# moxime/joint-vae

Hardware: AMD Instinct MI355X
Metric: training_images_per_sec (higher is better)
Workload: dtype f32

## Files before the change

include/jvae_hip.h:

```cpp
#ifndef JVAE_HIP_H
#define JVAE_HIP_H

#include <stddef.h>

#ifdef __cplusplus
extern "C" {
#endif

const char* jvae_version(void);

int jvae_gemm_f32(int M, int N, int K, int batch,
                  const float* A, long sAm, long sAk, long sAb,
                  const float* B, long sBk, long sBn, long sBb,
                  float* C, long sCm, long sCn, long sCb,
                  const float* bias, int bias_mode, int flags, int splitk, void* stream);

int jvae_splitk_fold_f32(const float* part, const float* bias, float* y, int S, long MN, int N, int relu, int accumulate,
                         void* stream);

size_t jvae_conv2d_workspace_bytes(int N, int Cin, int H, int W, int Cout, int KH, int KW, int S, int P, int OP,
                                   int transposed);
int jvae_conv2d_set_split_bf16(int mode);
int jvae_conv2d_set_split_shape16(int on);
int jvae_conv2d_out_shape(int H, int W, int KH, int KW, int S, int P, int OP, int transposed, int* OH, int* OW);
int jvae_conv2d_route(int dir, int layout, int bias, int stats, int y_f32, int aff_kind,
                      int N, int Cin, int H, int W, int Cout, int KH, int KW, int S, int P, int OP, int transposed,
                      int* kernel, int* swap, size_t* ws_bytes, int* splits, int* aff_ok);
const char* jvae_conv2d_kernel_name(int kernel);
int jvae_conv2d_fwd_f32(const float* x, const float* w, const float* bias, float* y,
                        int N, int Cin, int H, int W, int Cout, int KH, int KW, int S, int P, int OP, int transposed,
                        void* ws, size_t ws_bytes, void* stream);
int jvae_conv2d_stats_splits(int N, int Cin, int H, int W, int Cout, int KH, int KW, int S, int P, int OP, int transposed);
int jvae_conv2d_fwd_stats_f32(const float* x, const float* w, const float* bias, float* y, float* stats, int* nsplit,
                              int N, int Cin, int H, int W, int Cout, int KH, int KW, int S, int P, int OP, int transposed,
                              void* ws, size_t ws_bytes, void* stream);
int jvae_conv2d_dgrad_f32(const float* dy, const float* w, float* dx,
                          int N, int Cin, int H, int W, int Cout, int KH, int KW, int S, int P, int OP, int transposed,
                          void* ws, size_t ws_bytes, void* stream);
int jvae_conv2d_wgrad_f32(const float* x, const float* dy, float* dw, float* dbias, int accumulate,
                          int N, int Cin, int H, int W, int Cout, int KH, int KW, int S, int P, int OP, int transposed,
                          void* ws, size_t ws_bytes, void* stream);

int jvae_pack_cache_configure(void* buf, size_t bytes);
int jvae_pack_cache_begin(void* stream, long long owner, const void* const* weights, int n);
int jvae_pack_cache_end(void);
int jvae_pack_cache_pin(void);
int jvae_pack_cache_reset(void);
int jvae_pack_cache_stats(int* entries, long long* hits, long long* misses, long long* refreshes);

size_t jvae_channel_sum_workspace_bytes(int C);
int jvae_channel_sum_f32(const float* t, float* out, int N, int C, int P, int accumulate, void* ws, size_t ws_bytes,
                         void* stream);

size_t jvae_bn_workspace_bytes(int C);
int jvae_bn_plan(int N, int C, int P, int* nsplit, int* nchunk);
int jvae_image_range(int N, int parts, int j, int* nb, int* ne);
int jvae_bn_fwd_f32(const float* x, const float* gamma, const float* beta,
                    float* running_mean, float* running_var, long long* num_batches_tracked,
                    float* y, float* save_mean, float* save_invstd,
                    int N, int C, int P, float momentum, float eps, int training, int relu,
                    void* ws, size_t ws_bytes, void* stream);
int jvae_bn_fwd_ext_f32(const float* x, const float* gamma, const float* beta,
                        float* running_mean, float* running_var, long long* num_batches_tracked,
                        float* y, float* save_mean, float* save_invstd,
                        int N, int C, int P, float momentum, float eps, int training, int relu,
                        const float* ext_stats, int ext_nsplit, const float* ext_pivot,
                        void* ws, size_t ws_bytes, void* stream);
int jvae_bn_bwd_f32(const float* dy, const float* x, const float* gamma, const float* beta,
                    const float* save_mean, const float* save_invstd,
                    float* dx, float* dgamma, float* dbeta, int accumulate,
                    int N, int C, int P, int relu, void* ws, size_t ws_bytes, void* stream);
int jvae_bn_eval_bwd_f32(const float* dy, const float* x, const float* gamma, const float* beta,
                         const float* running_mean, const float* running_var, float* dx,
                         int N, int C, int P, float eps, int relu, void* stream);

int jvae_bn_finalize_f32(const float* x, const float* gamma, const float* beta,
                         float* running_mean, float* running_var, long long* num_batches_tracked,
                         float* save_mean, float* save_invstd, float* scale, float* shift,
                         int N, int C, int P, float momentum, float eps, int training,
                         const float* ext_stats, int ext_nsplit, const float* ext_pivot,
                         void* ws, size_t ws_bytes, void* stream);
int jvae_conv2d_affine_ok(int N, int Cin, int H, int W, int Cout, int KH, int KW, int S, int P, int OP, int transposed);
int jvae_conv2d_fwd_aff_f32(const float* x, const float* w, const float* bias, float* y, float* stats, int* nsplit,
                            const float* in_scale, const float* in_shift, int in_relu,
                            int N, int Cin, int H, int W, int Cout, int KH, int KW, int S, int P, int OP, int transposed,
                            void* ws, size_t ws_bytes, void* stream);
int jvae_conv2d_wgrad_aff_f32(const float* x, const float* dy, float* dw, float* dbias, int accumulate,
                              const float* in_scale, const float* in_shift, int in_relu,
                              int N, int Cin, int H, int W, int Cout, int KH, int KW, int S, int P, int OP, int transposed,
                              void* ws, size_t ws_bytes, void* stream);

int jvae_bn_sums_f32(const float* x, const float* pivot, float* sums, int N, int C, int P,
                     void* ws, size_t ws_bytes, void* stream);
int jvae_bn_fwd_sync_f32(const float* x, const float* gamma, const float* beta,
                         float* running_mean, float* running_var, long long* num_batches_tracked,
                         float* y, float* save_mean, float* save_invstd,
                         int N, int C, int P, float momentum, float eps, int relu,
                         const float* global_sums, const float* pivot, int world,
                         void* ws, size_t ws_bytes, void* stream);
int jvae_bn_bwd_sums_f32(const float* dy, const float* x, const float* gamma, const float* beta,
                         const float* save_mean, const float* save_invstd, float* local_sums,
                         int N, int C, int P, int relu, void* ws, size_t ws_bytes, void* stream);
int jvae_bn_bwd_sync_f32(const float* dy, const float* x, const float* gamma, const float* beta,
                         const float* save_mean, const float* save_invstd,
                         const float* local_sums, const float* global_sums, int world,
                         float* dx, float* dgamma, float* dbeta, int accumulate,
                         int N, int C, int P, int relu, void* stream);

int jvae_b8_pack_f32(const float* x, void* y, int N, int C, long HW, void* stream);
int jvae_b8_unpack_f32(const void* y, float* x, int N, int C, long HW, int accumulate, void* stream);
int jvae_conv2d_native_b8(int N, int Cin, int H, int W, int Cout, int KH, int KW, int S, int P, int OP, int transposed);
size_t jvae_conv2d_workspace_bytes_b8(int N, int Cin, int H, int W, int Cout, int KH, int KW, int S, int P, int OP,
                                      int transposed);
int jvae_conv2d_stats_splits_b8(int N, int Cin, int H, int W, int Cout, int KH, int KW, int S, int P, int OP, int transposed);
int jvae_conv2d_fwd_b8(const void* x, const float* w, const float* bias, void* y, int y_f32, float* stats, int* nsplit,
                       int N, int Cin, int H, int W, int Cout, int KH, int KW, int S, int P, int OP, int transposed,
                       void* ws, size_t ws_bytes, void* stream);
int jvae_conv2d_dgrad_b8(const void* dy, const float* w, void* dx,
                         int N, int Cin, int H, int W, int Cout, int KH, int KW, int S, int P, int OP, int transposed,
                         void* ws, size_t ws_bytes, void* stream);
int jvae_conv2d_wgrad_b8(const void* x, const void* dy, float* dw, float* dbias, int accumulate,
                         int N, int Cin, int H, int W, int Cout, int KH, int KW, int S, int P, int OP, int transposed,
                         void* ws, size_t ws_bytes, void* stream);
size_t jvae_bn_workspace_bytes_b8(int C);
int jvae_bn_plan_b8(int N, int C, long HW, int* nsplit, int* nchunk);
int jvae_bn_fwd_b8(const void* x, const float* gamma, const float* beta,
                   float* running_mean, float* running_var, long long* num_batches_tracked,
                   void* y, float* save_mean, float* save_invstd,
                   int N, int C, long HW, float momentum, float eps, int training, int relu,
                   const float* ext_stats, int ext_nsplit, const float* ext_pivot,
                   void* ws, size_t ws_bytes, void* stream);
int jvae_bn_bwd_b8(const void* dy, const void* x, const float* gamma, const float* beta,
                   const float* save_mean, const float* save_invstd,
                   void* dx, float* dgamma, float* dbeta, int accumulate,
                   int N, int C, long HW, int relu, void* ws, size_t ws_bytes, void* stream);
int jvae_bn_finalize_b8(const void* x, const float* gamma, const float* beta,
                        float* running_mean, float* running_var, long long* num_batches_tracked,
                        float* save_mean, float* save_invstd, float* coef,
                        int N, int C, long HW, float momentum, float eps, int training,
                        const float* ext_stats, int ext_nsplit, const float* ext_pivot,
                        void* ws, size_t ws_bytes, void* stream);
int jvae_bn_sums_b8(const void* x, const float* pivot, float* sums, int N, int C, long HW,
                    void* ws, size_t ws_bytes, void* stream);
int jvae_bn_fwd_sync_b8(const void* x, const float* gamma, const float* beta,
                        float* running_mean, float* running_var, long long* num_batches_tracked,
                        void* y, float* save_mean, float* save_invstd,
                        int N, int C, long HW, float momentum, float eps, int relu,
                        const float* global_sums, const float* pivot, int world,
                        void* ws, size_t ws_bytes, void* stream);
int jvae_bn_bwd_sums_b8(const void* dy, const void* x, const float* gamma, const float* beta,
                        const float* save_mean, const float* save_invstd, float* local_sums,
                        int N, int C, long HW, int relu, void* ws, size_t ws_bytes, void* stream);
int jvae_bn_bwd_sync_b8(const void* dy, const void* x, const float* gamma, const float* beta,
                        const float* save_mean, const float* save_invstd,
                        const float* local_sums, const float* global_sums, int world,
                        void* dx, float* dgamma, float* dbeta, int accumulate,
                        int N, int C, long HW, int relu, void* ws, size_t ws_bytes, void* stream);
int jvae_conv2d_affine_ok_b8(int N, int Cin, int H, int W, int Cout, int KH, int KW, int S, int P, int OP, int transposed);
int jvae_conv2d_fwd_aff_b8(const void* x, const float* w, const float* bias, void* y, int y_f32, float* stats, int* nsplit,
                           const float* in_scale, const float* in_shift, int in_relu,
                           int N, int Cin, int H, int W, int Cout, int KH, int KW, int S, int P, int OP, int transposed,
                           void* ws, size_t ws_bytes, void* stream);
int jvae_conv2d_wgrad_aff_b8(const void* x, const void* dy, float* dw, float* dbias, int accumulate,
                             const float* in_scale, const float* in_shift, int in_relu,
                             int N, int Cin, int H, int W, int Cout, int KH, int KW, int S, int P, int OP, int transposed,
                             void* ws, size_t ws_bytes, void* stream);
int jvae_relu_fwd_b8(const void* x, void* y, long units, void* stream);
int jvae_relu_bwd_b8(const void* dy, const void* y, void* dx, long units, void* stream);

int jvae_act_fwd_f32(const float* x, float* y, long n, int kind, void* stream);
int jvae_act_bwd_f32(const float* dy, const float* y, float* dx, long n, int kind, void* stream);

int jvae_dict_stats_f32(const float* means, float* dict, int C, int K, void* stream);
int jvae_latent_fwd_f32(const float* mu, const float* lv_raw, const float* eps, const long long* y,
                        const float* means, const float* T, const float* dict,
                        float* lv, float* z, float* kl, float* zdist, float* var_kl, float* dzdist,
                        int N, int K, int L, int C, int prior, int var_dim, float tau, float alpha, float w,
                        int sampled, int has_forced, float forced_lv, void* stream);
int jvae_latent_bwd_f32(const float* mu, const float* lv_raw, const float* lv, const float* eps, const long long* y,
                        const float* means, const float* T,
                        const float* gz, const float* g_kl, const float* g_zdist, const float* g_vkl,
                        const float* gmu_direct, const float* glv_direct,
                        float* gmu, float* glv_raw, float* gmeans, float* gT,
                        int N, int K, int L, int C, int prior, int var_dim, float tau, float alpha, float w,
                        int sampled, int has_forced, void* ws, size_t ws_bytes, void* stream);
int jvae_latent_fwd_wdev_f32(const float* mu, const float* lv_raw, const float* eps, const long long* y,
                             const float* means, const float* T, const float* dict,
                             float* lv, float* z, float* kl, float* zdist, float* var_kl, float* dzdist,
                             int N, int K, int L, int C, int prior, int var_dim, float tau, float alpha, float w,
                             int sampled, int has_forced, float forced_lv, const float* w_dev, void* stream);
int jvae_latent_bwd_wdev_f32(const float* mu, const float* lv_raw, const float* lv, const float* eps, const long long* y,
                             const float* means, const float* T,
                             const float* gz, const float* g_kl, const float* g_zdist, const float* g_vkl,
                             const float* gmu_direct, const float* glv_direct,
                             float* gmu, float* glv_raw, float* gmeans, float* gT,
                             int N, int K, int L, int C, int prior, int var_dim, float tau, float alpha, float w,
                             int sampled, int has_forced, const float* w_dev, void* ws, size_t ws_bytes, void* stream);
int jvae_latent_mixed_fwd_f32(const float* mu, const float* lv_raw, const float* eps, const long long* y,
                              const float* means_a, const float* T_a, const float* dict, const float* means_b, const float* T_b,
                              float* lv, float* z, float* kl, float* zdist, float* var_kl, float* dzdist,
                              int N, int K, int L, int split,
                              int C_a, int prior_a, int var_dim_a, float tau_a, float alpha_a,
                              int C_b, int prior_b, int var_dim_b, float tau_b, float alpha_b,
                              float w, int sampled, int has_forced, float forced_lv, void* stream);
int jvae_latent_mixed_bwd_f32(const float* mu, const float* lv_raw, const float* lv, const float* eps, const long long* y,
                              const float* means_a, const float* T_a, const float* means_b, const float* T_b,
                              const float* gz, const float* g_kl, const float* g_zdist, const float* g_vkl,
                              const float* gmu_direct, const float* glv_direct,
                              float* gmu, float* glv_raw, float* gmeans, float* gT,
                              int N, int K, int L, int split,
                              int C_a, int prior_a, int var_dim_a, float tau_a, float alpha_a,
                              int C_b, int prior_b, int var_dim_b, float tau_b, float alpha_b,
                              float w, int sampled, int has_forced, void* ws, size_t ws_bytes, void* stream);

int jvae_recon_fwd_f32(const float* x_reco, const float* x, const float* sigma, int sigma_is_log,
                       float* wmse, int L, int N, int D, void* stream);
int jvae_recon_bwd_f32(const float* x_reco, const float* x, const float* sigma, int sigma_is_log, const float* sigma_fwd,
                       const float* g_wmse, const float* wmse, float* g_x_reco, float* gsigma, int accumulate_sigma,
                       int L, int N, int D, void* ws, size_t ws_bytes, void* stream);

int jvae_mse_rows_fwd_f32(const float* rows, const float* x, float* wmse, int L, int N, int D, void* stream);
int jvae_mse_rows_bwd_f32(const float* rows, const float* x, const float* g_wmse, float* g_rows, int L, int N, int D, void* stream);

int jvae_elbo_fwd_f32(const float* wmse_s, const float* kl, const float* ce, const float* sigma, int sigma_is_log,
                      float* wmse, float* cross_x, float* total, float* mse, int L, int N, int D, float beta, float cw,
                      void* stream);
int jvae_elbo_bwd_f32(const float* g_wmse, const float* g_cx, const float* g_tot, const float* sigma, int sigma_is_log,
                      float* g_wmse_s, float* g_kl, float* g_ce, float* gsigma, int accumulate_sigma,
                      int L, int N, int D, float beta, float cw, void* ws, size_t ws_bytes, void* stream);
int jvae_elbo_fwd_wdev_f32(const float* wmse_s, const float* kl, const float* ce, const float* sigma, int sigma_is_log,
                           float* wmse, float* cross_x, float* total, float* mse, int L, int N, int D, float beta, float cw,
                           const float* cw_dev, void* stream);
int jvae_elbo_bwd_wdev_f32(const float* g_wmse, const float* g_cx, const float* g_tot, const float* sigma, int sigma_is_log,
                           float* g_wmse_s, float* g_kl, float* g_ce, float* gsigma, int accumulate_sigma,
                           int L, int N, int D, float beta, float cw, const float* cw_dev, void* ws, size_t ws_bytes,
                           void* stream);

int jvae_dropout_f32(const float* x, float* y, long n, float p, long seed, void* stream);
int jvae_dropout_dev_f32(const float* x, float* y, long n, float p, const long long* seed_dev, long salt, void* stream);

int jvae_iws_f32(const float* wmse_s, const float* eps, const float* log_var, const float* log_pz, const float* sigma,
                 int sigma_is_log, int L, int N, int K, int C, int D, float* rows, float* iws, void* stream);

int jvae_measures_f32(const float* sumsq_x, long nx, const float* wmse, const float* zdist, const float* var_kl, int N, int Nz,
                      const float* sigma, int sigma_is_log, const float* means, int C, int K, const int* flag,
                      const float* prev, int batch, float* out, void* stream);
int jvae_measures_dev_f32(const float* sumsq_x, long nx, const float* wmse, const float* zdist, const float* var_kl, int N, int Nz,
                          const float* sigma, int sigma_is_log, const float* means, int C, int K, const int* flag,
                          float* run, int* counter, void* stream);

int jvae_loss_sums_f32(const float* const* rows, const long* lens, int nrows, float* acc, void* stream);

int jvae_xent_fwd_f32(const float* logits, const long long* y, float* ce, int R, int N, int C, void* stream);
int jvae_xent_bwd_f32(const float* logits, const long long* y, const float* g_ce, float* g_logits, int R, int N, int C,
                      void* stream);

size_t jvae_sqnorm_workspace_bytes(void);
int jvae_sqnorm_accum_f32(const float* g, long n, float* acc, int reset, void* ws, size_t ws_bytes, void* stream);
int jvae_clip_scale_f32(float* g, long n, const float* sqnorm, float max_norm, void* stream);
int jvae_adam_step_f32(float* p, const float* g, float* m, float* v, long n,
                       float lr, float beta1, float beta2, float eps, float weight_decay, long step,
                       float max_norm, const float* sqnorm, int* nonfinite_flag, void* stream);
int jvae_adam_step_dev_f32(float* p, const float* g, float* m, float* v, long n, float* hyper, int advance,
                           float eps, float weight_decay, float max_norm, const float* sqnorm, int* nonfinite_flag,
                           void* stream);

int jvae_sgd_step_f32(float* p, const float* g, float* buf, long n, float lr, float momentum, int nesterov,
                      float weight_decay, int first_step, float max_norm, const float* sqnorm, int* nonfinite_flag,
                      void* stream);

int jvae_pool2d_out_shape(int H, int W, int K, int S, int P, int* OH, int* OW);
int jvae_pool2d_fwd_f32(const float* x, float* y, int* idx, long planes, int H, int W, int K, int S, int P, int mode,
                        void* stream);
int jvae_pool2d_bwd_f32(const float* dy, const int* idx, float* dx, long planes, int H, int W, int K, int S, int P,
                        int mode, void* stream);
int jvae_upsample_nearest_fwd_f32(const float* x, float* y, long planes, int H, int W, int scale, void* stream);
int jvae_upsample_nearest_bwd_f32(const float* dy, float* dx, long planes, int H, int W, int scale, void* stream);
int jvae_pool2d_fwd_b8(const void* x, void* y, int* idx, long blocks, int H, int W, int K, int S, int P, int mode, void* stream);
int jvae_pool2d_bwd_b8(const void* dy, const int* idx, void* dx, long blocks, int H, int W, int K, int S, int P, int mode,
                       void* stream);
int jvae_upsample_nearest_fwd_b8(const void* x, void* y, long blocks, int H, int W, int scale, void* stream);
int jvae_upsample_nearest_bwd_b8(const void* dy, void* dx, long blocks, int H, int W, int scale, void* stream);

int jvae_augment_u8_f32(const unsigned char* in, const unsigned char* flip, const int* dy, const int* dx,
                        float* out, int N, int C, int H, int W, int pad, int nhwc, void* stream);

int jvae_imageset_desc_words(void);
int jvae_imageset_batch_u8_f32(const unsigned char* data, const long long* idx, const long long* targets, const long long* lut,
                               const int* desc, const int* coef_h, const int* bounds_h, const int* coef_v, const int* bounds_v,
                               const unsigned char* flip, const int* dy, const int* dx, float* x, long long* y, long n, int N,
                               void* stream);

int jvae_imageset_mix_leaf_bytes(void);
int jvae_imageset_mixed_u8_f32(const void* leaves_host, const void* leaves_dev, int n_leaves, const int* leaf,
                               const long long* index, const long long* tag, const long long* pos, const float* u, int u_dims,
                               float* x, long long* tagout, long long* y, int N, int vec, void* stream);

size_t jvae_roc_workspace_bytes(int M, long n_in, long n_out);
int jvae_roc_curve_f32(const float* ins, const float* outs, const double* kept_tpr, const int* two_sided,
                       double* auc, double* kept_fpr, double* kept_tpr_out, double* thr_low, double* thr_up, int* status,
                       int M, long n_in, long n_out, int K, void* ws, size_t ws_bytes, void* stream);

int jvae_scod_scores_f32(const float* const* r_src, const float* const* r_aux, const float* const* g_src,
                         const float* const* g_alt, const int* kinds, const float* weights, const long long* y_est,
                         float* out, long out_stride, int M, int C, long N, int* status, void* stream);
size_t jvae_scod_workspace_bytes(int M, long n);
int jvae_scod_curve_f32(const float* scores, const long long* y_true, const long long* y_est, float* curves, double* figures,
                        int* status, int M, long n, long n_in, void* ws, size_t ws_bytes, void* stream);

int jvae_misclass_scores_f32(const float* src, const int* kinds, const float* temps, const int* rows, float* out,
                             int R, int C, long N, long out_stride, void* stream);
size_t jvae_misclass_split_workspace_bytes(long N);
int jvae_misclass_split_f32(const float* scores, const unsigned char* mask, float* out, int* n_correct, int M, long N,
                            void* ws, size_t ws_bytes, void* stream);
int jvae_misclass_confusion_f32(const float* scores, const unsigned char* mask, const double* thr, int* tp, int* fp,
                                int M, long N, int K, void* stream);

int jvae_odin_head_f32(const float* logits, const float* temps, float* scores, float* dlogits,
                       int F, int L, int N, int C, long stride_f, long stride_l, void* stream);
int jvae_odin_perturb_f32(float* acc, const float* g, const float* x, const float* eps, float* out, long numel, int E,
                          void* stream);
// ... 37 lines not shown
```

joint-vae_amd/csrc/gemm.hip:

```cpp
#include <stdlib.h>
#include "common.h"
#include "conv_x3.h"
#include "jvae_internal.h"
#include "conv_dispatch.h"

namespace {

constexpr int BK = 32;
constexpr int KQ = BK / 4;

struct GemmP {
    const float* A; long sAm, sAk, sAb;
    const float* B; long sBk, sBn, sBb;
    float* C; long sCm, sCn, sCb;
    const float* bias;
    int bias_mode;
    int bias_div;
    int M, N, K;
    int splitk;
    int kchunk;
    int flags;
    long sCsplit;
    int vecA, vecB;
    int xcd;
};

template <bool VEC>
__device__ __forceinline__ f32x4 load4(const float* p, long stride, int i0, int lim, bool row_ok) {
    f32x4 v = {0.f, 0.f, 0.f, 0.f};
    if (!row_ok) return v;
    if (VEC) {
        if (i0 + 3 < lim) return *reinterpret_cast<const f32x4*>(p);
    }
#pragma unroll
    for (int j = 0; j < 4; ++j)
        if (i0 + j < lim) v[j] = p[j * stride];
    return v;
}

template <int BM, int BN, bool AK, bool BNC>
__global__ __launch_bounds__(256) void gemm_kernel(GemmP p) {
    constexpr int LDA = BM + 4, LDB = BN + 4;
    constexpr int WM = BM / 2, WN = BN / 2;
    constexpr int TM = WM / 32, TN = WN / 32;
    constexpr int GA = BM * BK / 4 / 256;
    constexpr int GB = BN * BK / 4 / 256;
    __shared__ float As[BK * LDA];
    __shared__ float Bs[BK * LDB];

    const int tid = threadIdx.x, lane = tid & 63, wave = tid >> 6;
    const int wm0 = (wave >> 1) * WM, wn0 = (wave & 1) * WN;
    const int m0 = blockIdx.y * BM, n0 = blockIdx.x * BN;
    const int batch = blockIdx.z / p.splitk, split = blockIdx.z % p.splitk;
    const int kbeg = split * p.kchunk;
    const int kend = min(p.K, kbeg + p.kchunk);
    const float* A = p.A + (long)batch * p.sAb;
    const float* B = p.B + (long)batch * p.sBb;
    float* C = p.C + (long)batch * p.sCb + ((p.flags & 8) ? (long)split * p.sCsplit : 0L);

    f32x16 acc[TM][TN];
#pragma unroll
    for (int i = 0; i < TM; ++i)
#pragma unroll
        for (int j = 0; j < TN; ++j)
#pragma unroll
            for (int r = 0; r < 16; ++r) acc[i][j][r] = 0.f;

    f32x4 ra[GA], rb[GB];

    auto gload = [&](int k0) {
#pragma unroll
        for (int g = 0; g < GA; ++g) {
            if (AK) {
                const int kq = tid % KQ, row = tid / KQ + g * (256 / KQ);
                const int m = m0 + row, k = k0 + kq * 4;
                const float* src = A + (long)m * p.sAm + (long)k * p.sAk;
                ra[g] = p.vecA ? load4<true>(src, p.sAk, k, kend, m < p.M) : load4<false>(src, p.sAk, k, kend, m < p.M);
            } else {
                constexpr int GPR = BM / 4;
                const int mq = tid % GPR, kr = tid / GPR + g * (256 / GPR);
                const int m = m0 + mq * 4, k = k0 + kr;
                const float* src = A + (long)m * p.sAm + (long)k * p.sAk;
                ra[g] = p.vecA ? load4<true>(src, p.sAm, m, p.M, k < kend) : load4<false>(src, p.sAm, m, p.M, k < kend);
            }
        }
#pragma unroll
        for (int g = 0; g < GB; ++g) {
            if (BNC) {
                constexpr int GPR = BN / 4;
                const int nq = tid % GPR, kr = tid / GPR + g * (256 / GPR);
                const int n = n0 + nq * 4, k = k0 + kr;
                const float* src = B + (long)k * p.sBk + (long)n * p.sBn;
                rb[g] = p.vecB ? load4<true>(src, p.sBn, n, p.N, k < kend) : load4<false>(src, p.sBn, n, p.N, k < kend);
            } else {
                const int kq = tid % KQ, col = tid / KQ + g * (256 / KQ);
                const int n = n0 + col, k = k0 + kq * 4;
                const float* src = B + (long)k * p.sBk + (long)n * p.sBn;
                rb[g] = p.vecB ? load4<true>(src, p.sBk, k, kend, n < p.N) : load4<false>(src, p.sBk, k, kend, n < p.N);
            }
        }
    };
    auto lstore = [&]() {
#pragma unroll
        for (int g = 0; g < GA; ++g) {
            if (AK) {
                const int kq = tid % KQ, row = tid / KQ + g * (256 / KQ);
#pragma unroll
                for (int j = 0; j < 4; ++j) As[(kq * 4 + j) * LDA + row] = ra[g][j];
            } else {
                constexpr int GPR = BM / 4;
                const int mq = tid % GPR, kr = tid / GPR + g * (256 / GPR);
                *reinterpret_cast<f32x4*>(&As[kr * LDA + mq * 4]) = ra[g];
            }
        }
#pragma unroll
        for (int g = 0; g < GB; ++g) {
            if (BNC) {
                constexpr int GPR = BN / 4;
                const int nq = tid % GPR, kr = tid / GPR + g * (256 / GPR);
                *reinterpret_cast<f32x4*>(&Bs[kr * LDB + nq * 4]) = rb[g];
            } else {
                const int kq = tid % KQ, col = tid / KQ + g * (256 / KQ);
#pragma unroll
                for (int j = 0; j < 4; ++j) Bs[(kq * 4 + j) * LDB + col] = rb[g][j];
            }
        }
    };

    const int half = lane >> 5, l31 = lane & 31;
    if (kbeg < kend) gload(kbeg);
    for (int k0 = kbeg; k0 < kend; k0 += BK) {
        __syncthreads();
        lstore();
        __syncthreads();
        if (k0 + BK < kend) gload(k0 + BK);
#pragma unroll
        for (int kk = 0; kk < BK / 2; ++kk) {
            float a[TM], b[TN];
#pragma unroll
            for (int i = 0; i < TM; ++i) a[i] = As[(2 * kk + half) * LDA + wm0 + i * 32 + l31];
#pragma unroll
            for (int j = 0; j < TN; ++j) b[j] = Bs[(2 * kk + half) * LDB + wn0 + j * 32 + l31];
#pragma unroll
            for (int i = 0; i < TM; ++i)
#pragma unroll
                for (int j = 0; j < TN; ++j)
                    acc[i][j] = __builtin_amdgcn_mfma_f32_32x32x2f32(a[i], b[j], acc[i][j], 0, 0, 0);
        }
    }

    const bool lead = (split == 0) && !(p.flags & 8);
#pragma unroll
    for (int i = 0; i < TM; ++i)
#pragma unroll
        for (int j = 0; j < TN; ++j) {
            const int n = n0 + wn0 + j * 32 + l31;
            if (n >= p.N) continue;
            float bn = (p.bias_mode == 1 && lead) ? p.bias[n / p.bias_div] : 0.f;
#pragma unroll
            for (int r = 0; r < 16; ++r) {
                const int m = m0 + wm0 + i * 32 + (r & 3) + 8 * (r >> 2) + 4 * half;
                if (m >= p.M) continue;
                float v = acc[i][j][r] + bn;
                if (p.bias_mode == 2 && lead) v += p.bias[m];
                float* dst = C + (long)m * p.sCm + (long)n * p.sCn;
                if (p.flags & 8) {
                    *dst = v;
                } else if (p.flags & 4) {
                    atomicAdd(dst, v);
                } else {
                    if (p.flags & 1) v += *dst;
                    if (p.flags & 2) v = fmaxf(v, 0.f);
                    *dst = v;
                }
            }
        }
}

template <int BM, int BN>
int launch_tile(const GemmP& p, int batch, hipStream_t st) {
    dim3 grid(cdiv(p.N, BN), cdiv(p.M, BM), batch * p.splitk), block(256);
    const bool ak = (p.sAk == 1), bnc = (p.sBn == 1);
    if (ak && bnc)       hipLaunchKernelGGL((gemm_kernel<BM, BN, true, true>), grid, block, 0, st, p);
    else if (ak && !bnc) hipLaunchKernelGGL((gemm_kernel<BM, BN, true, false>), grid, block, 0, st, p);
    else if (!ak && bnc) hipLaunchKernelGGL((gemm_kernel<BM, BN, false, true>), grid, block, 0, st, p);
    else                 hipLaunchKernelGGL((gemm_kernel<BM, BN, false, false>), grid, block, 0, st, p);
    JVAE_LAUNCH_CHECK();
    return 0;
}

inline bool aligned16(const void* p) { return (reinterpret_cast<uintptr_t>(p) & 15) == 0; }

typedef __bf16 gx_bf16x8 __attribute__((ext_vector_type(8)));
typedef __bf16 gx_bf16x4 __attribute__((ext_vector_type(4)));
typedef unsigned int gx_u32x2 __attribute__((ext_vector_type(2)));
typedef unsigned int gx_u32x4 __attribute__((ext_vector_type(4)));
typedef __attribute__((address_space(3))) gx_bf16x4 gx_lds_bf16x4;
constexpr int BKX = 32;

__device__ __forceinline__ void gx_split4(const f32x4& v, gx_u32x2 (&out)[3]) {
#pragma unroll
    for (int j = 0; j < 2; ++j) {
        unsigned h, m, l;
        x3_split2(x3_f32x2{v[2 * j], v[2 * j + 1]}, h, m, l);
        out[0][j] = h; out[1][j] = m; out[2][j] = l;
    }
}

template <bool KC>
struct GxImg {
    static constexpr int PITCH = KC ? (BKX * 2 + 16) : (64 * 2 + 64);
    static constexpr int ROWS = KC ? 64 : BKX;
    static constexpr int BYTES = PITCH * ROWS;
};

template <bool AK, bool BNC, int DEPTH = 1>
__global__ __launch_bounds__(256, 4) void gemm_x3_kernel(GemmP p) {
    using IA = GxImg<AK>;
    using IB = GxImg<!BNC>;
    constexpr int BM = 64, BN = 64, G4 = BM * BKX / 4 / 256;
    constexpr int KQX = BKX / 4;
    extern __shared__ __attribute__((aligned(16))) unsigned char gx_lds[];
    unsigned char* As = gx_lds;
    unsigned char* Bs = gx_lds + 3 * IA::BYTES;

    const int tid = threadIdx.x, lane = tid & 63, wave = tid >> 6;
    const int half = lane >> 5, l31 = lane & 31;
    const int cg = (lane >> 4) & 1, q4 = (lane & 15) >> 2, pp = lane & 3;
    const int wm0 = (wave >> 1) * 32, wn0 = (wave & 1) * 32;
    unsigned bx = blockIdx.x, by = blockIdx.y, bz = blockIdx.z;
    if (p.xcd) {
        const unsigned lin = (unsigned)xcd_tile(bx + gridDim.x * (by + gridDim.y * bz), gridDim.x * gridDim.y * gridDim.z);
        bx = lin % gridDim.x; by = (lin / gridDim.x) % gridDim.y; bz = lin / (gridDim.x * gridDim.y);
    }
    const int m0 = by * BM, n0 = bx * BN;
    const int batch = bz / p.splitk, split = bz % p.splitk;
    const int kbeg = split * p.kchunk;
    const int kend = min(p.K, kbeg + p.kchunk);
    const float* A = p.A + (long)batch * p.sAb;
    const float* B = p.B + (long)batch * p.sBb;
    float* C = p.C + (long)batch * p.sCb + ((p.flags & 8) ? (long)split * p.sCsplit : 0L);

    f32x16 acc;
#pragma unroll
    for (int r = 0; r < 16; ++r) acc[r] = 0.f;
    f32x4 ra[DEPTH][G4], rb[DEPTH][G4];

    auto coordA = [&](int g, int k0, int* fast, int* slow) {
        if (AK) { *fast = k0 + (tid % KQX) * 4; *slow = m0 + tid / KQX + g * (256 / KQX); }
        else    { *fast = m0 + (tid % 16) * 4;  *slow = k0 + tid / 16 + g * 16; }
    };
    auto coordB = [&](int g, int k0, int* fast, int* slow) {
        if (BNC) { *fast = n0 + (tid % 16) * 4;  *slow = k0 + tid / 16 + g * 16; }
        else     { *fast = k0 + (tid % KQX) * 4; *slow = n0 + tid / KQX + g * (256 / KQX); }
    };
    auto okA = [&](int fast, int slow) { return AK ? (fast < kend && slow < p.M) : (fast + 3 < p.M && slow < kend); };
    auto okB = [&](int fast, int slow) { return BNC ? (fast + 3 < p.N && slow < kend) : (fast < kend && slow < p.N); };

    auto gload = [&](int st, int k0) {
#pragma unroll
        for (int g = 0; g < G4; ++g) {
            if constexpr (DEPTH > 1) {
                int f, sl;
                coordA(g, k0, &f, &sl);
                const float* sa = AK ? A + (long)sl * p.sAm + f : A + (long)sl * p.sAk + f;
                ra[st][g] = *reinterpret_cast<const f32x4*>(okA(f, sl) ? sa : A);
                coordB(g, k0, &f, &sl);
                const float* sb = BNC ? B + (long)sl * p.sBk + f : B + (long)sl * p.sBn + f;
                rb[st][g] = *reinterpret_cast<const f32x4*>(okB(f, sl) ? sb : B);
                continue;
            }
            if (AK) {
                const int kq = tid % KQX, row = tid / KQX + g * (256 / KQX);
                const int m = m0 + row, k = k0 + kq * 4;
                const float* src = A + (long)m * p.sAm + (long)k * p.sAk;
                ra[st][g] = p.vecA ? load4<true>(src, p.sAk, k, kend, m < p.M) : load4<false>(src, p.sAk, k, kend, m < p.M);
            } else {
                const int mq = tid % 16, kr = tid / 16 + g * 16;
                const int m = m0 + mq * 4, k = k0 + kr;
                const float* src = A + (long)m * p.sAm + (long)k * p.sAk;
                ra[st][g] = p.vecA ? load4<true>(src, p.sAm, m, p.M, k < kend) : load4<false>(src, p.sAm, m, p.M, k < kend);
            }
            if (BNC) {
                const int nq = tid % 16, kr = tid / 16 + g * 16;
                const int n = n0 + nq * 4, k = k0 + kr;
                const float* src = B + (long)k * p.sBk + (long)n * p.sBn;
                rb[st][g] = p.vecB ? load4<true>(src, p.sBn, n, p.N, k < kend) : load4<false>(src, p.sBn, n, p.N, k < kend);
            } else {
                const int kq = tid % KQX, col = tid / KQX + g * (256 / KQX);
                const int n = n0 + col, k = k0 + kq * 4;
                const float* src = B + (long)k * p.sBk + (long)n * p.sBn;
                rb[st][g] = p.vecB ? load4<true>(src, p.sBk, k, kend, n < p.N) : load4<false>(src, p.sBk, k, kend, n < p.N);
            }
        }
    };
    auto lstore = [&](int st, int k0) {
#pragma unroll
        for (int g = 0; g < G4; ++g) {
            const int fa = AK ? tid % KQX : tid % 16, sa_ = AK ? tid / KQX + g * (256 / KQX) : tid / 16 + g * 16;
            const int fb = BNC ? tid % 16 : tid % KQX, sb_ = BNC ? tid / 16 + g * 16 : tid / KQX + g * (256 / KQX);
            f32x4 va = ra[st][g], vb = rb[st][g];
            if constexpr (DEPTH > 1) {
                int f, sl;
                coordA(g, k0, &f, &sl);
                if (!okA(f, sl)) va = f32x4{0.f, 0.f, 0.f, 0.f};
                coordB(g, k0, &f, &sl);
                if (!okB(f, sl)) vb = f32x4{0.f, 0.f, 0.f, 0.f};
            }
            gx_u32x2 sa[3], sb[3];
            gx_split4(va, sa);
            gx_split4(vb, sb);
#pragma unroll
            for (int pl = 0; pl < 3; ++pl) {
                *reinterpret_cast<gx_u32x2*>(As + pl * IA::BYTES + sa_ * IA::PITCH + fa * 8) = sa[pl];
                *reinterpret_cast<gx_u32x2*>(Bs + pl * IB::BYTES + sb_ * IB::PITCH + fb * 8) = sb[pl];
            }
        }
    };
    auto frag = [&](const unsigned char* img, bool kc, int pitch, int r0, int ks) -> gx_bf16x8 {
        if (kc)
            return __builtin_bit_cast(gx_bf16x8, *reinterpret_cast<const gx_u32x4*>(img + (r0 + l31) * pitch + (ks * 16 + half * 8) * 2));
        const unsigned char* q = img + (ks * 16 + half * 8 + q4) * pitch + (r0 + cg * 16 + pp * 4) * 2;
        const gx_bf16x4 lo = __builtin_amdgcn_ds_read_tr16_b64_v4bf16((gx_lds_bf16x4*)q);
        const gx_bf16x4 hi = __builtin_amdgcn_ds_read_tr16_b64_v4bf16((gx_lds_bf16x4*)(q + 4 * pitch));
        return __builtin_shufflevector(lo, hi, 0, 1, 2, 3, 4, 5, 6, 7);
    };

    auto multiply = [&]() {
#pragma unroll
        for (int ks = 0; ks < BKX / 16; ++ks) {
            gx_bf16x8 a[3], b[3];
#pragma unroll
            for (int pl = 0; pl < 3; ++pl) {
                a[pl] = frag(As + pl * IA::BYTES, AK, IA::PITCH, wm0, ks);
                b[pl] = frag(Bs + pl * IB::BYTES, !BNC, IB::PITCH, wn0, ks);
            }
            constexpr int APL[6] = {0, 2, 1, 0, 1, 0}, BPL[6] = {2, 0, 1, 1, 0, 0};
#pragma unroll
            for (int t = 0; t < 6; ++t) acc = __builtin_amdgcn_mfma_f32_32x32x16_bf16(a[APL[t]], b[BPL[t]], acc, 0, 0, 0);
        }
    };
    if constexpr (DEPTH > 1) {
#pragma unroll
        for (int d = 0; d < DEPTH; ++d) gload(d, kbeg + d * BKX);
        const int nst = (kend - kbeg + BKX - 1) / BKX;
        int k0 = kbeg;
        for (int it = 0; it < nst / DEPTH; ++it, k0 += DEPTH * BKX) {
#pragma unroll
            for (int d = 0; d < DEPTH; ++d) {
                const int kk = k0 + d * BKX;
                __syncthreads();
                lstore(d, kk);
                __syncthreads();
                gload(d, kk + DEPTH * BKX);
                multiply();
            }
        }
#pragma unroll
        for (int d = 0; d < DEPTH - 1; ++d) {
            const int kk = k0 + d * BKX;
            if (kk < kend) {
                __syncthreads();
                lstore(d, kk);
                __syncthreads();
                multiply();
            }
        }
    } else {
        if (kbeg < kend) gload(0, kbeg);
        for (int k0 = kbeg; k0 < kend; k0 += BKX) {
            __syncthreads();
            lstore(0, k0);
            __syncthreads();
            if (k0 + BKX < kend) gload(0, k0 + BKX);
            multiply();
        }
    }

    const bool lead = (split == 0) && !(p.flags & 8);
    const int n = n0 + wn0 + l31;
    if (n >= p.N) return;
    const float bn = (p.bias_mode == 1 && lead) ? p.bias[n / p.bias_div] : 0.f;
#pragma unroll
    for (int r = 0; r < 16; ++r) {
        const int m = m0 + wm0 + (r & 3) + 8 * (r >> 2) + 4 * half;
        if (m >= p.M) continue;
        float v = acc[r] + bn;
        if (p.bias_mode == 2 && lead) v += p.bias[m];
        float* dst = C + (long)m * p.sCm + (long)n * p.sCn;
        if (p.flags & 8) {
            *dst = v;
        } else if (p.flags & 4) {
            atomicAdd(dst, v);
        } else {
            if (p.flags & 1) v += *dst;
            if (p.flags & 2) v = fmaxf(v, 0.f);
            *dst = v;
        }
    }
}

template <bool AK, bool BNC, int DEPTH>
int launch_x3_variant(const GemmP& p, int batch, hipStream_t st) {
    constexpr int LDS = 3 * (GxImg<AK>::BYTES + GxImg<!BNC>::BYTES);
    static bool attr_set = false;
    if (!attr_set) {
        hipError_t e = hipFuncSetAttribute(reinterpret_cast<const void*>(&gemm_x3_kernel<AK, BNC, DEPTH>),
                                           hipFuncAttributeMaxDynamicSharedMemorySize, LDS);
        if (e != hipSuccess) return (int)e;
        attr_set = true;
    }
    dim3 grid(cdiv(p.N, 64), cdiv(p.M, 64), batch * p.splitk), block(256);
    hipLaunchKernelGGL((gemm_x3_kernel<AK, BNC, DEPTH>), grid, block, LDS, st, p);
    JVAE_LAUNCH_CHECK();
    return 0;
}

template <bool AK, bool BNC>
int launch_x3_ab(const GemmP& p, int batch, hipStream_t st) {
    const bool deep = p.vecA && p.vecB && p.K % 4 == 0
                      && (AK || p.M % 4 == 0) && (!BNC || p.N % 4 == 0);
    if (deep) return launch_x3_variant<AK, BNC, 3>(p, batch, st);
    return launch_x3_variant<AK, BNC, 1>(p, batch, st);
}

int launch_x3(const GemmP& p0, int batch, hipStream_t st) {
    GemmP p = p0;
    p.xcd = 1;
    const bool ak = (p.sAk == 1), bnc = (p.sBn == 1);
    if (ak && bnc) return launch_x3_ab<true, true>(p, batch, st);
    if (ak) return launch_x3_ab<true, false>(p, batch, st);
    if (bnc) return launch_x3_ab<false, true>(p, batch, st);
    return launch_x3_ab<false, false>(p, batch, st);
}

inline bool gemm_x3_on(int K) {
    return K >= 64 && jvae_conv5_x3_enabled();
}

}

int jvae_gemm_launch(int M, int N, int K, int batch,
                     const float* A, long sAm, long sAk, long sAb,
                     const float* B, long sBk, long sBn, long sBb,
                     float* C, long sCm, long sCn, long sCb,
                     const float* bias, int bias_mode, int flags, int splitk, hipStream_t st) {
    return jvae_gemm_launch_ex(M, N, K, batch, A, sAm, sAk, sAb, B, sBk, sBn, sBb, C, sCm, sCn, sCb, bias, bias_mode, 1,
                               flags, splitk, st);
}

int jvae_gemm_launch_ex(int M, int N, int K, int batch,
                        const float* A, long sAm, long sAk, long sAb,
                        const float* B, long sBk, long sBn, long sBb,
                        float* C, long sCm, long sCn, long sCb,
                        const float* bias, int bias_mode, int bias_div, int flags, int splitk, hipStream_t st) {
    if (M <= 0 || N <= 0 || batch <= 0) return 0;
    if (K < 0 || !A || !B || !C) return JVAE_EINVAL;
    if (bias_mode && !bias) return JVAE_EINVAL;
    GemmP p;
    p.A = A; p.sAm = sAm; p.sAk = sAk; p.sAb = sAb;
    p.B = B; p.sBk = sBk; p.sBn = sBn; p.sBb = sBb;
    p.C = C; p.sCm = sCm; p.sCn = sCn; p.sCb = sCb;
    p.bias = bias; p.bias_mode = bias_mode; p.bias_div = bias_div > 0 ? bias_div : 1;
    p.M = M; p.N = N; p.K = K;
    if (splitk < 1) splitk = 1;
    int ktiles = cdiv(K, BK);
    if (splitk > ktiles) splitk = ktiles > 0 ? ktiles : 1;
    p.kchunk = cdiv(ktiles, splitk) * BK;
    splitk = K > 0 ? cdiv(K, p.kchunk) : 1;
    p.splitk = splitk;
    p.flags = flags & ~8;
    p.sCsplit = 0;
    if (splitk > 1) {
        if (flags & 2) return JVAE_EINVAL;
        p.flags |= 4;
    }
    const bool ak = (sAk == 1), bnc = (sBn == 1);
    p.vecA = aligned16(A) && (sAb % 4 == 0) && (ak ? (sAm % 4 == 0) : (sAm == 1 && sAk % 4 == 0));
    p.vecB = aligned16(B) && (sBb % 4 == 0) && (bnc ? (sBk % 4 == 0) : (sBk == 1 && sBn % 4 == 0));
    if (gemm_x3_on(K)) return launch_x3(p, batch, st);
    const long tiles128 = (long)cdiv(M, 128) * cdiv(N, 128) * batch * splitk;
    if (M > 64 && N > 64 && tiles128 >= 512) return launch_tile<128, 128>(p, batch, st);
    return launch_tile<64, 64>(p, batch, st);
}

int jvae_gemm_launch_part(int M, int N, int K, int batch,
                          const float* A, long sAm, long sAk, long sAb,
                          const float* B, long sBk, long sBn, long sBb,
                          float* part, long sCm, long sCn, long sCb, long sCsplit, int want_splits, int* splits,
                          hipStream_t st) {
    if (splits) *splits = 0;
    if (M <= 0 || N <= 0 || batch <= 0) return 0;
    if (K <= 0 || !A || !B || !part || !splits) return JVAE_EINVAL;
    GemmP p;
    p.A = A; p.sAm = sAm; p.sAk = sAk; p.sAb = sAb;
    p.B = B; p.sBk = sBk; p.sBn = sBn; p.sBb = sBb;
    p.C = part; p.sCm = sCm; p.sCn = sCn; p.sCb = sCb;
    p.bias = nullptr; p.bias_mode = 0; p.bias_div = 1;
    p.M = M; p.N = N; p.K = K;
    int splitk = want_splits < 1 ? 1 : want_splits;
    const int ktiles = cdiv(K, BK);
    if (splitk > ktiles) splitk = ktiles;
    p.kchunk = cdiv(ktiles, splitk) * BK;
    splitk = cdiv(K, p.kchunk);
    p.splitk = splitk;
    p.flags = 8;
    p.sCsplit = sCsplit;
    const bool ak = (sAk == 1), bnc = (sBn == 1);
    p.vecA = aligned16(A) && (sAb % 4 == 0) && (ak ? (sAm % 4 == 0) : (sAm == 1 && sAk % 4 == 0));
    p.vecB = aligned16(B) && (sBb % 4 == 0) && (bnc ? (sBk % 4 == 0) : (sBk == 1 && sBn % 4 == 0));
    *splits = splitk;
    if (gemm_x3_on(K)) return launch_x3(p, batch, st);
    return launch_tile<64, 64>(p, batch, st);
}

__global__ __launch_bounds__(256) void splitk_fold_kernel(const float* __restrict__ part, const float* __restrict__ bias,
                                                          float* __restrict__ y, int S, long MN, int N, int relu,
                                                          int accumulate, int bias_div) {
    for (long i = (long)blockIdx.x * blockDim.x + threadIdx.x; i < MN; i += (long)gridDim.x * blockDim.x) {
        float v = bias ? bias[(i / bias_div) % N] : 0.f;
        for (int s = 0; s < S; ++s) v += part[(long)s * MN + i];
        if (accumulate) v += y[i];
        y[i] = relu ? fmaxf(v, 0.f) : v;
    }
}

__global__ __launch_bounds__(256) void splitk_fold_qn_kernel(const float* __restrict__ part, const float* __restrict__ bias,
                                                             float* __restrict__ y, int S, int N, int Cs, int Ps) {
    const long total = (long)Ps * N * Cs;
    for (long i = (long)blockIdx.x * blockDim.x + threadIdx.x; i < total; i += (long)gridDim.x * blockDim.x) {
        const int cs = (int)(i % Cs);
        const long r = i / Cs;
        const int n = (int)(r % N), q = (int)(r / N);
        float v = bias ? bias[cs] : 0.f;
        for (int s = 0; s < S; ++s) v += part[(long)s * total + i];
        y[((long)n * Cs + cs) * Ps + q] = v;
    }
}

int jvae_splitk_fold_qn(const float* part, const float* bias, float* y, int S, int N, int Cs, int Ps, hipStream_t st) {
    const long total = (long)Ps * N * Cs;
    if (total == 0) return 0;
    const int blocks = (int)((total + 255) / 256 > 4096 ? 4096 : (total + 255) / 256);
    hipLaunchKernelGGL(splitk_fold_qn_kernel, dim3(blocks), dim3(256), 0, st, part, bias, y, S, N, Cs, Ps);
    JVAE_LAUNCH_CHECK();
    return 0;
}

int jvae_splitk_fold(const float* part, const float* bias, float* y, int S, long MN, int N, int relu, int accumulate,
                     hipStream_t st, int bias_div) {
    if (MN == 0) return 0;
    const int blocks = (int)((MN + 255) / 256 > 4096 ? 4096 : (MN + 255) / 256);
    hipLaunchKernelGGL(splitk_fold_kernel, dim3(blocks), dim3(256), 0, st, part, bias, y, S, MN, N, relu, accumulate,
                       bias_div > 0 ? bias_div : 1);
    JVAE_LAUNCH_CHECK();
    return 0;
}

extern "C" int jvae_splitk_fold_f32(const float* part, const float* bias, float* y, int S, long MN, int N, int relu,
                                    int accumulate, void* stream) {
    if (!part || !y || S < 1 || MN < 0 || N < 1) return JVAE_EINVAL;
    return jvae_splitk_fold(part, bias, y, S, MN, N, relu, accumulate, (hipStream_t)stream);
}

extern "C" int jvae_gemm_f32(int M, int N, int K, int batch,
                             const float* A, long sAm, long sAk, long sAb,
                             const float* B, long sBk, long sBn, long sBb,
                             float* C, long sCm, long sCn, long sCb,
                             const float* bias, int bias_mode, int flags, int splitk, void* stream) {
    return jvae_gemm_launch(M, N, K, batch, A, sAm, sAk, sAb, B, sBk, sBn, sBb, C, sCm, sCn, sCb,
                            bias, bias_mode, flags, splitk, (hipStream_t)stream);
}
```

joint-vae_amd/jvae_hip/lib.py:

```python
import ctypes
import os
from ctypes import c_char_p, c_float, c_int, c_long, c_longlong, c_size_t, c_void_p, POINTER

import torch

_HERE = os.path.dirname(os.path.abspath(__file__))
LIB_PATH = os.environ.get('JVAE_HIP_LIB') or os.path.join(_HERE, 'libjvae_hip.so')

_lib = None

P = c_void_p
_SIGS = {
    'jvae_version': (c_char_p, []),
    'jvae_gemm_f32': (c_int, [c_int] * 4 + [P, c_long, c_long, c_long] * 3 + [P, c_int, c_int, c_int, P]),
    'jvae_splitk_fold_f32': (c_int, [P, P, P, c_int, c_long, c_int, c_int, c_int, P]),
    'jvae_conv2d_workspace_bytes': (c_size_t, [c_int] * 11),
    'jvae_conv2d_set_split_bf16': (c_int, [c_int]),
    'jvae_conv2d_set_split_shape16': (c_int, [c_int]),
    'jvae_conv2d_out_shape': (c_int, [c_int] * 8 + [POINTER(c_int), POINTER(c_int)]),
    'jvae_conv2d_route': (c_int, [c_int] * 17 + [POINTER(c_int), POINTER(c_int), POINTER(c_size_t), POINTER(c_int), POINTER(c_int)]),
    'jvae_conv2d_kernel_name': (c_char_p, [c_int]),
    'jvae_conv2d_fwd_f32': (c_int, [P, P, P, P] + [c_int] * 11 + [P, c_size_t, P]),
    'jvae_conv2d_stats_splits': (c_int, [c_int] * 11),
    'jvae_conv2d_fwd_stats_f32': (c_int, [P, P, P, P, P, POINTER(c_int)] + [c_int] * 11 + [P, c_size_t, P]),
    'jvae_conv2d_dgrad_f32': (c_int, [P, P, P] + [c_int] * 11 + [P, c_size_t, P]),
    'jvae_conv2d_wgrad_f32': (c_int, [P, P, P, P, c_int] + [c_int] * 11 + [P, c_size_t, P]),
    'jvae_b8_pack_f32': (c_int, [P, P, c_int, c_int, c_long, P]),
    'jvae_b8_unpack_f32': (c_int, [P, P, c_int, c_int, c_long, c_int, P]),
    'jvae_conv2d_native_b8': (c_int, [c_int] * 11),
    'jvae_conv2d_workspace_bytes_b8': (c_size_t, [c_int] * 11),
    'jvae_conv2d_stats_splits_b8': (c_int, [c_int] * 11),
    'jvae_conv2d_fwd_b8': (c_int, [P, P, P, P, c_int, P, POINTER(c_int)] + [c_int] * 11 + [P, c_size_t, P]),
    'jvae_conv2d_dgrad_b8': (c_int, [P, P, P] + [c_int] * 11 + [P, c_size_t, P]),
    'jvae_conv2d_wgrad_b8': (c_int, [P, P, P, P, c_int] + [c_int] * 11 + [P, c_size_t, P]),
    'jvae_bn_workspace_bytes_b8': (c_size_t, [c_int]),
    'jvae_bn_plan_b8': (c_int, [c_int, c_int, c_long, POINTER(c_int), POINTER(c_int)]),
    'jvae_bn_fwd_b8': (c_int, [P] * 9 + [c_int, c_int, c_long, c_float, c_float, c_int, c_int, P, c_int, P, P, c_size_t, P]),
    'jvae_bn_bwd_b8': (c_int, [P] * 9 + [c_int, c_int, c_int, c_long, c_int, P, c_size_t, P]),
    'jvae_bn_finalize_b8': (c_int, [P] * 9 + [c_int, c_int, c_long, c_float, c_float, c_int, P, c_int, P, P, c_size_t, P]),
    'jvae_bn_sums_b8': (c_int, [P, P, P, c_int, c_int, c_long, P, c_size_t, P]),
    'jvae_bn_fwd_sync_b8': (c_int, [P] * 9 + [c_int, c_int, c_long, c_float, c_float, c_int, P, P, c_int, P, c_size_t, P]),
    'jvae_bn_bwd_sums_b8': (c_int, [P] * 7 + [c_int, c_int, c_long, c_int, P, c_size_t, P]),
    'jvae_bn_bwd_sync_b8': (c_int, [P] * 8 + [c_int, P, P, P, c_int, c_int, c_int, c_long, c_int, P, c_size_t, P]),
    'jvae_conv2d_affine_ok_b8': (c_int, [c_int] * 11),
    'jvae_conv2d_fwd_aff_b8': (c_int, [P, P, P, P, c_int, P, POINTER(c_int), P, P, c_int] + [c_int] * 11 + [P, c_size_t, P]),
    'jvae_conv2d_wgrad_aff_b8': (c_int, [P, P, P, P, c_int, P, P, c_int] + [c_int] * 11 + [P, c_size_t, P]),
    'jvae_relu_fwd_b8': (c_int, [P, P, c_long, P]),
    'jvae_relu_bwd_b8': (c_int, [P, P, P, c_long, P]),
    'jvae_bn_finalize_f32': (c_int, [P] * 10 + [c_int, c_int, c_int, c_float, c_float, c_int, P, c_int, P, P, c_size_t, P]),
    'jvae_conv2d_affine_ok': (c_int, [c_int] * 11),
    'jvae_conv2d_fwd_aff_f32': (c_int, [P, P, P, P, P, POINTER(c_int), P, P, c_int] + [c_int] * 11 + [P, c_size_t, P]),
    'jvae_conv2d_wgrad_aff_f32': (c_int, [P, P, P, P, c_int, P, P, c_int] + [c_int] * 11 + [P, c_size_t, P]),
    'jvae_pack_cache_configure': (c_int, [P, c_size_t]),
    'jvae_pack_cache_begin': (c_int, [P, c_longlong, P, c_int]),
    'jvae_pack_cache_end': (c_int, []),
    'jvae_pack_cache_pin': (c_int, []),
    'jvae_pack_cache_reset': (c_int, []),
    'jvae_pack_cache_stats': (c_int, [POINTER(c_int), POINTER(c_longlong), POINTER(c_longlong), POINTER(c_longlong)]),
    'jvae_channel_sum_workspace_bytes': (c_size_t, [c_int]),
    'jvae_channel_sum_f32': (c_int, [P, P, c_int, c_int, c_int, c_int, P, c_size_t, P]),
    'jvae_bn_workspace_bytes': (c_size_t, [c_int]),
    'jvae_bn_plan': (c_int, [c_int, c_int, c_int, POINTER(c_int), POINTER(c_int)]),
    'jvae_image_range': (c_int, [c_int, c_int, c_int, POINTER(c_int), POINTER(c_int)]),
    'jvae_bn_fwd_f32': (c_int, [P] * 9 + [c_int, c_int, c_int, c_float, c_float, c_int, c_int, P, c_size_t, P]),
    'jvae_bn_fwd_ext_f32': (c_int, [P] * 9 + [c_int, c_int, c_int, c_float, c_float, c_int, c_int, P, c_int, P, P, c_size_t, P]),
    'jvae_bn_sums_f32': (c_int, [P, P, P, c_int, c_int, c_int, P, c_size_t, P]),
    'jvae_bn_fwd_sync_f32': (c_int, [P] * 9 + [c_int, c_int, c_int, c_float, c_float, c_int, P, P, c_int, P, c_size_t, P]),
    'jvae_bn_bwd_sums_f32': (c_int, [P] * 7 + [c_int, c_int, c_int, c_int, P, c_size_t, P]),
    'jvae_bn_bwd_sync_f32': (c_int, [P] * 8 + [c_int, P, P, P, c_int, c_int, c_int, c_int, c_int, P]),
    'jvae_bn_bwd_f32': (c_int, [P] * 9 + [c_int, c_int, c_int, c_int, c_int, P, c_size_t, P]),
    'jvae_bn_eval_bwd_f32': (c_int, [P] * 7 + [c_int, c_int, c_int, c_float, c_int, P]),
    'jvae_act_fwd_f32': (c_int, [P, P, c_long, c_int, P]),
    'jvae_act_bwd_f32': (c_int, [P, P, P, c_long, c_int, P]),
    'jvae_dict_stats_f32': (c_int, [P, P, c_int, c_int, P]),
    'jvae_latent_fwd_f32': (c_int, [P] * 13 + [c_int] * 6 + [c_float] * 3 + [c_int, c_int, c_float, P]),
    'jvae_latent_bwd_f32': (c_int, [P] * 17 + [c_int] * 6 + [c_float] * 3 + [c_int, c_int, P, c_size_t, P]),
    'jvae_latent_fwd_wdev_f32': (c_int, [P] * 13 + [c_int] * 6 + [c_float] * 3 + [c_int, c_int, c_float, P, P]),
    'jvae_latent_bwd_wdev_f32': (c_int, [P] * 17 + [c_int] * 6 + [c_float] * 3 + [c_int, c_int, P, P, c_size_t, P]),
    'jvae_latent_mixed_fwd_f32': (c_int, [P] * 15 + [c_int] * 4 + ([c_int] * 3 + [c_float] * 2) * 2
                                  + [c_float, c_int, c_int, c_float, P]),
    'jvae_latent_mixed_bwd_f32': (c_int, [P] * 19 + [c_int] * 4 + ([c_int] * 3 + [c_float] * 2) * 2
                                  + [c_float, c_int, c_int, P, c_size_t, P]),
    'jvae_recon_fwd_f32': (c_int, [P, P, P, c_int, P, c_int, c_int, c_int, P]),
    'jvae_recon_bwd_f32': (c_int, [P, P, P, c_int, P, P, P, P, P, c_int, c_int, c_int, c_int, P, c_size_t, P]),
    'jvae_mse_rows_fwd_f32': (c_int, [P, P, P, c_int, c_int, c_int, P]),
    'jvae_mse_rows_bwd_f32': (c_int, [P, P, P, P, c_int, c_int, c_int, P]),
    'jvae_elbo_fwd_f32': (c_int, [P, P, P, P, c_int, P, P, P, P, c_int, c_int, c_int, c_float, c_float, P]),
    'jvae_elbo_bwd_f32': (c_int, [P, P, P, P, c_int, P, P, P, P, c_int, c_int, c_int, c_int, c_float, c_float, P, c_size_t, P]),
    'jvae_elbo_fwd_wdev_f32': (c_int, [P, P, P, P, c_int, P, P, P, P, c_int, c_int, c_int, c_float, c_float, P, P]),
    'jvae_elbo_bwd_wdev_f32': (c_int, [P, P, P, P, c_int, P, P, P, P, c_int, c_int, c_int, c_int, c_float, c_float, P, P, c_size_t, P]),
    'jvae_measures_dev_f32': (c_int, [P, c_long, P, P, P, c_int, c_int, P, c_int, P, c_int, c_int, P, P, P, P]),
    'jvae_loss_sums_f32': (c_int, [P, P, c_int, P, P]),
    'jvae_measures_f32': (c_int, [P, c_long, P, P, P, c_int, c_int, P, c_int, P, c_int, c_int, P, P, c_int, P, P]),
    'jvae_dropout_f32': (c_int, [P, P, c_long, c_float, c_long, P]),
    'jvae_dropout_dev_f32': (c_int, [P, P, c_long, c_float, P, c_long, P]),
    'jvae_iws_f32': (c_int, [P, P, P, P, P, c_int, c_int, c_int, c_int, c_int, c_int, P, P, P]),
    'jvae_xent_fwd_f32': (c_int, [P, P, P, c_int, c_int, c_int, P]),
    'jvae_xent_bwd_f32': (c_int, [P, P, P, P, c_int, c_int, c_int, P]),
    'jvae_augment_u8_f32': (c_int, [P, P, P, P, P, c_int, c_int, c_int, c_int, c_int, c_int, P]),
    'jvae_imageset_desc_words': (c_int, []),
    'jvae_imageset_batch_u8_f32': (c_int, [P] * 4 + [POINTER(c_int)] + [P] * 9 + [c_long, c_int, P]),
    'jvae_imageset_mix_leaf_bytes': (c_int, []),
    'jvae_imageset_mixed_u8_f32': (c_int, [P, P, c_int] + [P] * 5 + [c_int] + [P] * 3 + [c_int, c_int, P]),
    'jvae_sqnorm_workspace_bytes': (c_size_t, []),
    'jvae_sqnorm_accum_f32': (c_int, [P, c_long, P, c_int, P, c_size_t, P]),
    'jvae_clip_scale_f32': (c_int, [P, c_long, P, c_float, P]),
    'jvae_adam_step_dev_f32': (c_int, [P, P, P, P, c_long, P, c_int, c_float, c_float, c_float, P, P, P]),
    'jvae_adam_step_f32': (c_int, [P, P, P, P, c_long] + [c_float] * 5 + [c_long, c_float, P, P, P]),
    'jvae_sgd_step_f32': (c_int, [P, P, P, c_long, c_float, c_float, c_int, c_float, c_int, c_float, P, P, P]),
    'jvae_pool2d_out_shape': (c_int, [c_int] * 5 + [POINTER(c_int), POINTER(c_int)]),
    'jvae_pool2d_fwd_f32': (c_int, [P, P, P, c_long] + [c_int] * 6 + [P]),
    'jvae_pool2d_bwd_f32': (c_int, [P, P, P, c_long] + [c_int] * 6 + [P]),
    'jvae_upsample_nearest_fwd_f32': (c_int, [P, P, c_long, c_int, c_int, c_int, P]),
    'jvae_upsample_nearest_bwd_f32': (c_int, [P, P, c_long, c_int, c_int, c_int, P]),
    'jvae_pool2d_fwd_b8': (c_int, [P, P, P, c_long] + [c_int] * 6 + [P]),
    'jvae_pool2d_bwd_b8': (c_int, [P, P, P, c_long] + [c_int] * 6 + [P]),
    'jvae_upsample_nearest_fwd_b8': (c_int, [P, P, c_long, c_int, c_int, c_int, P]),
    'jvae_upsample_nearest_bwd_b8': (c_int, [P, P, c_long, c_int, c_int, c_int, P]),
    'jvae_roc_workspace_bytes': (c_size_t, [c_int, c_long, c_long]),
    'jvae_roc_curve_f32': (c_int, [P] * 10 + [c_int, c_long, c_long, c_int, P, c_size_t, P]),
    'jvae_scod_scores_f32': (c_int, [P] * 8 + [c_long, c_int, c_int, c_long, P, P]),
    'jvae_scod_workspace_bytes': (c_size_t, [c_int, c_long]),
    'jvae_scod_curve_f32': (c_int, [P] * 6 + [c_int, c_long, c_long, P, c_size_t, P]),
    'jvae_misclass_scores_f32': (c_int, [P] * 5 + [c_int, c_int, c_long, c_long, P]),
    'jvae_misclass_split_workspace_bytes': (c_size_t, [c_long]),
    'jvae_misclass_split_f32': (c_int, [P, P, P, P, c_int, c_long, P, c_size_t, P]),
    'jvae_misclass_confusion_f32': (c_int, [P] * 5 + [c_int, c_long, c_int, P]),
    'jvae_odin_head_f32': (c_int, [P, P, P, P, c_int, c_int, c_int, c_int, c_long, c_long, P]),
    'jvae_odin_perturb_f32': (c_int, [P, P, P, P, P, c_long, c_int, P]),
    'jvae_wim_scores_f32': (c_int, [P, P, P, c_int, P, P, c_int, P, c_long, c_int, c_long, P, P]),
    'jvae_group_tally_f32': (c_int, [P, P, P, P, c_int, c_int, c_int, P]),
    'jvae_prior_sample_f32': (c_int, [P] * 6 + [c_long, c_int, c_int, c_float, c_int, P]),
    'jvae_image_grid_f32': (c_int, [P, P, P, P, c_int, P, P] + [c_int] * 5 + [P]),
    'jvae_class_posterior_f32': (c_int, [P] * 5 + [c_int, P, P, c_long, c_int, c_int, c_int, P]),
    'jvae_latent_mi_workspace_bytes': (c_size_t, [c_int, c_int, c_long]),
    'jvae_latent_mi_f32': (c_int, [P, P, P, c_int, c_int, c_int, c_int, c_long, P, c_size_t, P]),
    'jvae_aggregate_scores_f32': (c_int, [P, P, c_int, c_int, P, c_int, P, P, P, P, c_int, c_int, c_long, P, P]),
    'jvae_cascade_mse_workspace_bytes': (c_size_t, [c_int, c_long, c_long]),
    'jvae_cascade_mse_f32': (c_int, [P, P, c_int, P, c_int, c_long, c_long, P, c_size_t, P]),
    'jvae_iterate_prior_f32': (c_int, [P, P, c_int, c_int, c_long, P]),
    'jvae_latent_moments_workspace_bytes': (c_size_t, [c_int, c_int, c_int]),
    'jvae_latent_moments_f32': (c_int, [P, P, P, P, P, c_int, c_int, c_int, P, c_size_t, P]),
    'jvae_nearest_centroid_f32': (c_int, [P, P, P, P, c_long, c_int, c_int, P]),
    'jvae_histogram_f32': (c_int, [P, P, P, P, P, c_long, c_int, c_int, P]),
}


class JvaeHipError(RuntimeError):
    pass


def load():
    global _lib
    if _lib is not None:
        return _lib
    if not os.path.exists(LIB_PATH):
        raise JvaeHipError(f'{LIB_PATH} is missing: build it with `python -c "import __graft_entry__ as g; g.build()"` '
                           'or `make -C joint-vae_amd/csrc` (there is no CPU/PyTorch fallback)')
    lib = ctypes.CDLL(LIB_PATH)
    for name, (res, args) in _SIGS.items():
        fn = getattr(lib, name)
        fn.restype = res
        fn.argtypes = args
    _lib = lib
    return lib


def exported_symbols():
    return list(_SIGS)


_ERR = {-1: 'invalid argument', -2: 'unsupported configuration', -3: 'workspace too small'}


def check(rc, what):
    if rc != 0:
        msg = _ERR.get(rc, f'hipError_t {rc}')
        raise JvaeHipError(f'{what} failed: {msg}')


_raw_stream = getattr(torch._C, '_cuda_getCurrentRawStream', None)


def stream_ptr(device_index=None):
    if _raw_stream is not None:
        return _raw_stream(torch.cuda.current_device() if device_index is None else device_index)
    return torch.cuda.current_stream().cuda_stream


def ptr(t):
    if t is None:
        return None
    if not t.is_cuda:
        raise JvaeHipError('jvae_hip ops need tensors resident on the GPU (no CPU fallback); got device '
                           + str(t.device))
    if not t.is_contiguous():
        raise JvaeHipError('jvae_hip ops need contiguous tensors')
    return t.data_ptr()


_workspaces = {}
_side_streams = {}


def side_stream(device):
    idx = device.index if device.index is not None else torch.cuda.current_device()
    st = _side_streams.get(idx)
    if st is None:
        _side_streams[idx] = st = torch.cuda.Stream(device=idx)
    return st


def join_side_stream(device=None):
    for idx, st in _side_streams.items():
        if device is None or device.index in (None, idx):
            torch.cuda.current_stream(idx).wait_stream(st)


def workspace(nbytes, device):
    idx = device.index if device.index is not None else torch.cuda.current_device()
    key = (idx, stream_ptr(idx))
    ws = _workspaces.get(key)
    if ws is None or ws.numel() < nbytes:
        _workspaces[key] = ws = torch.empty(max(int(nbytes), 1 << 20), dtype=torch.uint8, device=device)
    return ws


PACK_CACHE_BYTES = int(os.environ.get('JVAE_PACK_CACHE_MB', '64')) << 20
_pack_cache = {}
span_depth = 0
span_hold = 0


def pack_cache_begin(weights, device):
    if not PACK_CACHE_BYTES:
        return
    lib = load()
    idx = device.index if device.index is not None else torch.cuda.current_device()
    if idx not in _pack_cache:
        if _pack_cache:
            check(lib.jvae_pack_cache_configure(None, 0), 'jvae_pack_cache_configure')
            _pack_cache[idx] = None
        else:
            buf = torch.empty(PACK_CACHE_BYTES + 256, dtype=torch.uint8, device=device)
            off = (-buf.data_ptr()) % 256
            _pack_cache[idx] = buf
            check(lib.jvae_pack_cache_configure(buf.data_ptr() + off, PACK_CACHE_BYTES), 'jvae_pack_cache_configure')
    if _pack_cache[idx] is None:
        return
    addrs = tuple(w.data_ptr() for w in weights)
    arr = (ctypes.c_void_p * max(len(addrs), 1))(*addrs)
    check(lib.jvae_pack_cache_begin(stream_ptr(idx), hash(addrs), arr, len(addrs)), 'jvae_pack_cache_begin')


def pack_cache_end():
    if _lib is not None and _pack_cache:
        _lib.jvae_pack_cache_end()


def pack_cache_pin():
    if _lib is not None and _pack_cache and PACK_CACHE_BYTES:
        _lib.jvae_pack_cache_pin()


def pack_cache_stats():
    lib = load()
    e, h, m, r = c_int(), c_longlong(), c_longlong(), c_longlong()
    lib.jvae_pack_cache_stats(ctypes.byref(e), ctypes.byref(h), ctypes.byref(m), ctypes.byref(r))
    return {'entries': e.value, 'hits': h.value, 'misses': m.value, 'refreshes': r.value}
```

joint-vae_amd/jvae_hip/ops.py:

```python
import collections
import contextlib
import ctypes
import math
from ctypes import byref, c_int, c_size_t

import numpy as np
import torch

from . import lib as L

RELU, SIGMOID, IDENT, LEAKY = 1, 2, 0, 3
BN_ACT = {IDENT: 0, RELU: 1, LEAKY: 2}
OVERLAP_WGRAD = True
ACT_KIND = {'relu': RELU, 'sigmoid': SIGMOID, 'linear': IDENT, 'leaky': LEAKY, None: IDENT}


def _c(t):
    return t if t.is_contiguous() else t.contiguous()


def _f32(t, what):
    if t.dtype != torch.float32:
        raise L.JvaeHipError(f'{what}: fp32 expected, got {t.dtype}')
    return t


def _grad_slot(param):
    if param is None or not isinstance(param, torch.nn.Parameter):
        return None
    g = param.grad
    if g is None or not g.is_contiguous() or g.dtype != torch.float32 or g.shape != param.shape or not g.is_cuda:
        return None
    return g


def _join_after_backward():
    torch.autograd.Variable._execution_engine.queue_callback(L.join_side_stream)


def _close_span_after_backward():
    if not L.span_hold:
        torch.autograd.Variable._execution_engine.queue_callback(L.pack_cache_end)


def gemm(M, N, K, A, sA, B, sB, C, sC, bias=None, bias_mode=0, flags=0, splitk=1, batch=1):
    lib = L.load()
    rc = lib.jvae_gemm_f32(M, N, K, batch, L.ptr(A), *sA, L.ptr(B), *sB, L.ptr(C), *sC,
                           L.ptr(bias), bias_mode, flags, splitk, L.stream_ptr())
    L.check(rc, 'jvae_gemm_f32')


def channel_sum(t, N, C, P, out=None, accumulate=False):
    lib = L.load()
    if out is None:
        out = torch.empty(C, device=t.device, dtype=torch.float32)
    ws = L.workspace(lib.jvae_channel_sum_workspace_bytes(C), t.device)
    L.check(lib.jvae_channel_sum_f32(L.ptr(t), L.ptr(out), N, C, P, int(accumulate), L.ptr(ws), ws.numel(), L.stream_ptr()),
            'channel_sum')
    return out


def _linear_split(R, O, I):
    tiles = ((R + 63) // 64) * ((O + 63) // 64)
    if tiles >= 128 or I < 512:
        return 1
    for S in (32, 16, 8, 4, 2):
        if tiles * S <= 1024 and I % S == 0 and I // S >= 128:
            return S
    return 1


class _Linear(torch.autograd.Function):

    @staticmethod
    def forward(ctx, x, w, b, act):
        x2 = _c(_f32(x, 'linear').reshape(-1, x.shape[-1]))
        w_in = w
        w = _c(w)
        R, I = x2.shape
        O = w.shape[0]
        y = torch.empty((R, O), device=x.device, dtype=torch.float32)
        S = _linear_split(R, O, I)
        if S > 1:
            part = torch.empty((S, R, O), device=x.device, dtype=torch.float32)
            Ks = I // S
            gemm(R, O, Ks, x2, (I, 1, Ks), w, (1, I, Ks), part, (O, 1, R * O), batch=S)
            L.check(L.load().jvae_splitk_fold_f32(L.ptr(part), L.ptr(b), L.ptr(y), S, R * O, O, int(act == RELU), 0,
                                                  L.stream_ptr()), 'jvae_splitk_fold_f32')
        else:
            gemm(R, O, I, x2, (I, 1, 0), w, (1, I, 0), y, (O, 1, 0), bias=b, bias_mode=1 if b is not None else 0,
                 flags=2 if act == RELU else 0)
        if act in (SIGMOID, LEAKY):
            L.check(L.load().jvae_act_fwd_f32(L.ptr(y), L.ptr(y), y.numel(), act, L.stream_ptr()), 'act_fwd')
        ctx.save_for_backward(x2, w, y if act != IDENT else None)
        ctx.act = act
        ctx.has_bias = b is not None
        ctx.xshape = x.shape
        ctx.w_ref, ctx.b_ref = w_in, b
        return y.reshape(*x.shape[:-1], O)

    @staticmethod
    def backward(ctx, gy):
        x2, w, y = ctx.saved_tensors
        lib = L.load()
        R, I = x2.shape
        O = w.shape[0]
        gy = _c(gy.reshape(R, O))
        if ctx.act != IDENT:
            g = torch.empty_like(gy)
            L.check(lib.jvae_act_bwd_f32(L.ptr(gy), L.ptr(y), L.ptr(g), gy.numel(), ctx.act, L.stream_ptr()), 'act_bwd')
            gy = g
        gx = gw = gb = None
        if ctx.needs_input_grad[0]:
            gx = torch.empty((R, I), device=gy.device, dtype=torch.float32)
            gemm(R, I, O, gy, (O, 1, 0), w, (I, 1, 0), gx, (I, 1, 0))
            gx = gx.reshape(ctx.xshape)
        if ctx.needs_input_grad[1]:
            slot = _grad_slot(ctx.w_ref)
            gw = slot if slot is not None else torch.zeros((O, I), device=gy.device, dtype=torch.float32)
            S = _linear_split(O, I, R)
            if S > 1:
                part = torch.empty((S, O, I), device=gy.device, dtype=torch.float32)
                Rs = R // S
                gemm(O, I, Rs, gy, (1, O, Rs * O), x2, (I, 1, Rs * I), part, (I, 1, O * I), batch=S)
                L.check(lib.jvae_splitk_fold_f32(L.ptr(part), None, L.ptr(gw), S, O * I, I, 0, 1, L.stream_ptr()),
                        'jvae_splitk_fold_f32')
            else:
                gemm(O, I, R, gy, (1, O, 0), x2, (I, 1, 0), gw, (I, 1, 0), flags=1)
            if slot is not None:
                gw = None
        if ctx.has_bias and ctx.needs_input_grad[2]:
            slot = _grad_slot(ctx.b_ref)
            if slot is not None:
                channel_sum(gy, R, O, 1, out=slot, accumulate=True)
            else:
                gb = channel_sum(gy, R, O, 1)
        return gx, gw, gb, None


def linear(x, w, b=None, act=IDENT):
    return _Linear.apply(x, w, b, act)


_GEOM_CACHE = {}


def _geom_query(name, geom):
    key = (name, geom)
    r = _GEOM_CACHE.get(key)
    if r is None:
        _GEOM_CACHE[key] = r = getattr(L.load(), name)(*geom)
    return r


class ConvSpec:
    __slots__ = ('cin', 'cout', 'k', 's', 'p', 'op', 'transposed')

    def __init__(self, cin, cout, k, s, p, op=0, transposed=False):
        self.cin, self.cout, self.k, self.s, self.p, self.op, self.transposed = cin, cout, k, s, p, op, bool(transposed)

    def out_hw(self, H, W):
        key = ('hw', self.k, self.s, self.p, self.op, self.transposed, H, W)
        r = _GEOM_CACHE.get(key)
        if r is None:
            oh, ow = c_int(), c_int()
            rc = L.load().jvae_conv2d_out_shape(H, W, self.k, self.k, self.s, self.p, self.op, int(self.transposed),
                                                byref(oh), byref(ow))
            L.check(rc, 'jvae_conv2d_out_shape')
            _GEOM_CACHE[key] = r = (oh.value, ow.value)
        return r

    def geom(self, N, H, W):
        return (N, self.cin, H, W, self.cout, self.k, self.k, self.s, self.p, self.op, int(self.transposed))


def _conv_ws(geom, device):
    nbytes = _geom_query('jvae_conv2d_workspace_bytes', geom)
    ws = L.workspace(nbytes, device)
    return ws, ws.numel()


def conv_fwd_raw(x, w, b, spec):
    N, _, H, W = x.shape
    oh, ow = spec.out_hw(H, W)
    y = torch.empty((N, spec.cout, oh, ow), device=x.device, dtype=torch.float32)
    geom = spec.geom(N, H, W)
    ws, nb = _conv_ws(geom, x.device)
    rc = L.load().jvae_conv2d_fwd_f32(L.ptr(x), L.ptr(w), L.ptr(b), L.ptr(y), *geom, L.ptr(ws), nb, L.stream_ptr())
    L.check(rc, 'jvae_conv2d_fwd_f32')
    return y


def conv_fwd_stats_raw(x, w, b, spec):
    lib = L.load()
    N, _, H, W = x.shape
    geom = spec.geom(N, H, W)
    cap = _geom_query('jvae_conv2d_stats_splits', geom)
    if cap <= 0:
        return conv_fwd_raw(x, w, b, spec), None, 0
    oh, ow = spec.out_hw(H, W)
    y = torch.empty((N, spec.cout, oh, ow), device=x.device, dtype=torch.float32)
    stats = torch.empty((spec.cout * cap * 2,), device=x.device, dtype=torch.float32)
    ws, nb = _conv_ws(geom, x.device)
    ns = c_int(0)
    rc = lib.jvae_conv2d_fwd_stats_f32(L.ptr(x), L.ptr(w), L.ptr(b), L.ptr(y), L.ptr(stats), byref(ns), *geom,
                                       L.ptr(ws), nb, L.stream_ptr())
    L.check(rc, 'jvae_conv2d_fwd_stats_f32')
    return y, (stats if ns.value > 0 else None), ns.value


def conv_affine_ok(spec, N, H, W):
    return bool(_geom_query('jvae_conv2d_affine_ok', spec.geom(N, H, W)))


ConvRoute = collections.namedtuple('ConvRoute', 'kernel swap ws splits aff_ok')
ROUTE_DIR = {'fwd': 1, 'dgrad': 2, 'wgrad': 4}
ROUTE_LAYOUT = {'f32': 0, 'b8': 1}


def conv_route(spec, N, H, W, direction, layout='f32', bias=False, stats=False, y_f32=False, aff=0):
    lib = L.load()
    k, sw, ns, ok, ws = c_int(), c_int(), c_int(), c_int(), c_size_t()
    rc = lib.jvae_conv2d_route(ROUTE_DIR[direction], ROUTE_LAYOUT[layout], int(bias), int(stats), int(y_f32), int(aff),
                               *spec.geom(N, H, W), byref(k), byref(sw), byref(ws), byref(ns), byref(ok))
    L.check(rc, 'jvae_conv2d_route')
    return ConvRoute(lib.jvae_conv2d_kernel_name(k.value).decode(), bool(sw.value), ws.value, ns.value, bool(ok.value))


class LaunchProbe:

    def __init__(self, match):
        self.match, self.events, self.armed = match, [], False

    def times_ms(self):
        return [a.elapsed_time(b) for a, b in self.events]


FWD_AFF_PROBE = None


def conv_fwd_aff_raw(x, w, b, spec, aff, want_stats):
    lib = L.load()
    N, _, H, W = x.shape
    geom = spec.geom(N, H, W)
    oh, ow = spec.out_hw(H, W)
    y = torch.empty((N, spec.cout, oh, ow), device=x.device, dtype=torch.float32)
    stats, ns = None, c_int(0)
    if want_stats:
        cap = _geom_query('jvae_conv2d_stats_splits', geom)
        if cap > 0:
            stats = torch.empty((spec.cout * cap * 2,), device=x.device, dtype=torch.float32)
    ws, nb = _conv_ws(geom, x.device)
    probe = FWD_AFF_PROBE
    timed = probe is not None and probe.armed and probe.match(spec, N, H)
    if timed:
        ev = (torch.cuda.Event(enable_timing=True), torch.cuda.Event(enable_timing=True))
        ev[0].record()
    rc = lib.jvae_conv2d_fwd_aff_f32(L.ptr(x), L.ptr(w), L.ptr(b), L.ptr(y), L.ptr(stats), byref(ns),
                                     L.ptr(aff[0]), L.ptr(aff[1]), int(aff[2]), *geom, L.ptr(ws), nb, L.stream_ptr())
    if timed:
        ev[1].record()
        probe.events.append(ev)
    L.check(rc, 'jvae_conv2d_fwd_aff_f32')
    return y, (stats if ns.value > 0 else None), ns.value


def conv_dgrad_raw(gy, w, spec, xshape):
    N, _, H, W = xshape
    gx = torch.empty(xshape, device=gy.device, dtype=torch.float32)
    geom = spec.geom(N, H, W)
    ws, nb = _conv_ws(geom, gy.device)
    rc = L.load().jvae_conv2d_dgrad_f32(L.ptr(gy), L.ptr(w), L.ptr(gx), *geom, L.ptr(ws), nb, L.stream_ptr())
    L.check(rc, 'jvae_conv2d_dgrad_f32')
    return gx


def conv_wgrad_raw(x, gy, spec, wshape, want_bias, w_slot=None, b_slot=None, aff=None):
    N, _, H, W = x.shape
    inplace = w_slot is not None and (b_slot is not None or not want_bias)
    gw = w_slot if inplace else torch.empty(wshape, device=x.device, dtype=torch.float32)
    gb = None
    if want_bias:
        gb = b_slot if inplace else torch.empty(spec.cout, device=x.device, dtype=torch.float32)
    geom = spec.geom(N, H, W)
    ws, nb = _conv_ws(geom, x.device)
    if aff is not None:
        rc = L.load().jvae_conv2d_wgrad_aff_f32(L.ptr(x), L.ptr(gy), L.ptr(gw), L.ptr(gb), int(inplace),
                                                L.ptr(aff[0]), L.ptr(aff[1]), int(aff[2]), *geom, L.ptr(ws), nb,
                                                L.stream_ptr())
    else:
        rc = L.load().jvae_conv2d_wgrad_f32(L.ptr(x), L.ptr(gy), L.ptr(gw), L.ptr(gb), int(inplace), *geom, L.ptr(ws), nb,
                                            L.stream_ptr())
    L.check(rc, 'jvae_conv2d_wgrad_f32')
    return (None, None) if inplace else (gw, gb)


FWD, DGRAD, WGRAD = 1, 2, 4


class Layout:
    sfx = '_f32'
    ws_sfx = ''
    acts = BN_ACT

    def dims(self, x, C):
        N, C = x.shape[0], x.shape[1]
        return N, C, x.numel() // max(N * C, 1)

    def coef_width(self, C):
        return C

    def prep(self, x, what):
        return _c(_f32(x, what))

    def to_f32(self, t, C):
        return t

    def from_f32(self, t):
        return t

    def native(self, spec, N, H, W):
        return FWD | DGRAD | WGRAD

    def affine_ok(self, spec, N, H, W):
        return conv_affine_ok(spec, N, H, W)

    def conv_fwd(self, x, w, b, spec, want_stats, aff, out_f32):
        if aff is not None:
            return conv_fwd_aff_raw(x, w, b, spec, aff, want_stats)
        if want_stats:
            return conv_fwd_stats_raw(x, w, b, spec)
        return conv_fwd_raw(x, w, b, spec), None, 0

    def conv_dgrad(self, gy, w, spec, N, H, W):
        return conv_dgrad_raw(gy, w, spec, (N, spec.cin, H, W))

    def conv_wgrad(self, *args):
        return conv_wgrad_raw(*args)

    def bn(self, name, *args, ws=None):
        name += self.sfx
        extra = () if ws is None else (L.ptr(ws), ws.numel())
        L.check(getattr(L.load(), name)(*args, *extra, L.stream_ptr()), name)

    def bn_workspace(self, C, device):
        return L.workspace(getattr(L.load(), 'jvae_bn_workspace_bytes' + self.ws_sfx)(C), device)

    def bn_fwd(self, *args, ext, ws):
        if ext[0] is None:
            self.bn('jvae_bn_fwd', *args, ws=ws)
        else:
            self.bn('jvae_bn_fwd_ext', *args, *ext, ws=ws)

    def coef_args(self, coef):
        return L.ptr(coef[0]), L.ptr(coef[1])

    def bn_bwd_sync(self, *args, ws):
        self.bn('jvae_bn_bwd_sync', *args)


F32 = Layout()


def layout_of(t):
    return _b8.B8 if _b8.is_b8(t) else F32


class _Conv(torch.autograd.Function):

    @staticmethod
    def forward(ctx, x, w, b, spec, dead_bias, stats_out, aff, out_f32):
        lay = layout_of(x)
        x = lay.prep(x, 'conv')
        if not L.span_depth:
            L.pack_cache_end()
        ctx.w_ref, ctx.b_ref = w, b
        w = _c(w)
        native = lay.native(spec, x.shape[0], x.shape[2], x.shape[3])
        if aff is not None and (native & (FWD | WGRAD)) != FWD | WGRAD:
            raise L.JvaeHipError('a deferred BatchNorm needs native forward and weight-gradient kernels (conv_affine_ok)')
        want_stats = stats_out is not None
        if native & FWD:
            y, st, ns = lay.conv_fwd(x, w, b, spec, want_stats, aff, out_f32)
        else:
            y, st, ns = F32.conv_fwd(lay.to_f32(x, spec.cin), w, b, spec, want_stats, None, False)
            y = y if out_f32 else lay.from_f32(y)
        if want_stats:
            stats_out['stats'], stats_out['nsplit'], stats_out['pivot'] = st, ns, b
        ctx.save_for_backward(x, w)
        ctx.lay, ctx.native, ctx.spec, ctx.out_f32, ctx.aff = lay, native, spec, out_f32, aff
        ctx.has_bias = b is not None
        ctx.dead_bias = dead_bias
        return y

    @staticmethod
    def backward(ctx, gy):
        x, w = ctx.saved_tensors
        lay, spec = ctx.lay, ctx.spec
        N, H, W = x.shape[0], x.shape[2], x.shape[3]
        gys = {F32 if ctx.out_f32 else lay: _c(gy)}

        def gy_in(want):
            if want not in gys:
                have, g = next(iter(gys.items()))
                gys[want] = want.from_f32(g) if have is F32 else have.to_f32(g, spec.cout)
            return gys[want]
        gx = gw = gb = None
        _close_span_after_backward()
        want_b = ctx.has_bias and ctx.needs_input_grad[2] and not ctx.dead_bias
        wgrad = ctx.needs_input_grad[1] or want_b
        on_side = False
        if wgrad:
            w_slot = _grad_slot(ctx.w_ref)
            b_slot = _grad_slot(ctx.b_ref) if want_b else None
            on_side = (OVERLAP_WGRAD and ctx.needs_input_grad[0] and w_slot is not None
                       and (b_slot is not None or not want_b))
        if ctx.needs_input_grad[0]:
            dl = lay if ctx.native & DGRAD else F32
            gyd = gy_in(dl)
        if on_side:
            side = L.side_stream(x.device)
            side.wait_stream(torch.cuda.current_stream(x.device))
        if ctx.needs_input_grad[0]:
            gx = dl.conv_dgrad(gyd, w, spec, N, H, W)
            gx = gx if dl is lay else lay.from_f32(gx)
        if wgrad:
            with torch.cuda.stream(side) if on_side else contextlib.nullcontext():
                wl = lay if ctx.native & WGRAD else F32
                xw = x if wl is lay else lay.to_f32(x, spec.cin)
                gw, gb = wl.conv_wgrad(xw, gy_in(wl), spec, w.shape, want_b, w_slot, b_slot, ctx.aff)
            if on_side:
                for t in (x, xw, *gys.values(), *(ctx.aff[:2] if ctx.aff is not None else ())):
                    t.record_stream(side)
                _join_after_backward()
        if ctx.dead_bias and ctx.has_bias and ctx.needs_input_grad[2] and _grad_slot(ctx.b_ref) is None:
            gb = torch.zeros_like(ctx.b_ref)
        return gx, gw, gb, None, None, None, None, None


def conv2d(x, w, b, spec, dead_bias=False, stats_out=None, aff=None, out_f32=False):
    return _Conv.apply(x, w, b, spec, dead_bias, stats_out, aff, out_f32)


def _ext_args(ext, training):
# ... 1624 lines not shown
```

joint-vae_amd/module/vae_layers/layers.py:

```python
import logging
import math

import numpy as np
import torch
from torch import nn
from torch.nn import Parameter

from jvae_hip import ops
from jvae_compat import texify_str
from module.priors import build_prior
from .misc import activation_layers, ACT_OF_MODULE


def _sigma_kind(is_rmse, coded, learned, decay):
    for kind, on in (('rmse', is_rmse), ('coded', coded), ('learned', learned), ('decayed', decay)):
        if on:
            return kind
    return 'fixed'


class Sigma(Parameter):

    @staticmethod
    def __new__(cls, value=None, sdim=1, input_dim=False, learned=False, is_rmse=False, is_log=False, **_):
        if value is None:
            assert is_rmse or input_dim, 'a Sigma needs a value unless it follows the rmse or is coded'
        stored_as_log = bool(is_log or learned or input_dim)
        if is_rmse or (input_dim and value is None):
            start = 0.
        else:
            start = float(value)
        shape = (sdim,) if isinstance(sdim, int) else tuple(sdim)
        with np.errstate(divide='ignore'):
            init = float(np.log(start)) if stored_as_log else start
        return super().__new__(cls, torch.full(shape, init), requires_grad=bool(learned or input_dim))

    def __init__(self, value=None, learned=False, is_rmse=False, sdim=1, input_dim=False, reach=1, decay=0,
                 max_step=None, sigma0=None, is_log=False):
        if learned:
            assert not is_rmse and not decay, 'a learned sigma neither follows the rmse nor decays'
        follows = bool(decay) or is_rmse
        public = dict(is_rmse=is_rmse,
                      sigma0=sigma0 if (sigma0 is not None or is_rmse) else value,
                      learned=learned,
                      input_dim=input_dim,
                      is_log=learned or is_log or input_dim,
                      decay=1 if is_rmse else decay,
                      reach=reach if follows else None,
                      max_step=max_step,
                      sdim=sdim)
        self._rmse = np.nan
        self.__dict__.update(public)
        self._output_dim = None
        if input_dim:
            self._output_dim = input_dim if sdim != 1 else (1,) * len(input_dim)

    def __deepcopy__(self, memo):
        twin = Sigma.__new__(Sigma, value=1.0, sdim=self.sdim, learned=self.requires_grad)
        twin.__dict__.update(self.__dict__)
        twin.data = self.data.clone()
        memo[id(self)] = twin
        return twin

    coded = property(lambda self: bool(self.input_dim))
    per_dim = property(lambda self: self.sdim != 1)
    output_dim = property(lambda self: self._output_dim)
    kind = property(lambda self: _sigma_kind(self.is_rmse, self.coded, self.learned, self.decay))

    @property
    def value(self):
        with torch.no_grad():
            squares = (2 * self.data).exp() if self.is_log else self.data * self.data
            return float(squares.mean().sqrt())

    def host_params(self, value):
        listed = {k: v for k, v in vars(self).items() if k[:1] != '_'}
        listed['value'] = value
        return listed

    @property
    def params(self):
        return self.host_params(self.value)

    def update(self, rmse=None, v=None):
        assert rmse is None or v is None
        if v is not None:
            extra = v.dim() - self.dim()
            assert extra >= 0
            self.data = v.mean(tuple(range(extra))) if extra else v
        elif rmse is not None:
            self._rmse = rmse
            if self.kind in ('rmse', 'decayed'):
                step = self.decay * (self.reach * rmse - self.data)
                if self.max_step:
                    step = torch.clamp(torch.as_tensor(step), -self.max_step, self.max_step)
                self.data += step

    def _describe(self):
        kind = self.kind
        if kind == 'rmse':
            return 'rmse' if self._rmse is np.nan else 'rmse ({:g})'.format(self._rmse)
        if kind == 'coded':
            return 'coded ' + ('mask' if self.per_dim else 'scalar')
        if kind == 'learned':
            return '{:g}->rmse[l] ({:g})'.format(self.sigma0, self.value)
        if kind == 'fixed':
            return '{:g}'.format(self.value if self.dim() and self.numel() > 1 else float(self.data))
        target = ('' if self.reach == 1 else '{:g}*'.format(self.reach)) + 'rmse'
        limit = '<{:g}'.format(self.max_step) if self.max_step else ''
        return '{:g}->{}[-{:g}*{}]'.format(self.sigma0, target, self.decay, limit)

    def __str__(self):
        return self._describe()

    def __format__(self, spec):
        tail = spec[-1:] if spec else ''
        if tail in ('f', 'g', 'e'):
            return format(self.value, spec)
        if tail == 'x':
            return texify_str(self._describe(), num=True)
        if tail == 'i':
            letter = {'rmse': 'e', 'learned': 'l', 'coded': 'C' if self.per_dim else 'c'}.get(self.kind)
            if letter:
                return letter
        return self._describe()

    def __repr__(self):
        if self.kind == 'rmse':
            return 'Sigma will be RMSE'
        text = super().__repr__()
        if self.decay:
            text = '{}, decaying to {}*mse with rate {})'.format(text[:-1], self.reach, self.decay)
        return text


def draw_epsilon(sampling_size, shape, device, distribution='gaussian'):
    size = (sampling_size + 1,) + tuple(shape)
    if distribution == 'gaussian':
        eps = torch.randn(size, device=device)
    else:
        eps = (torch.rand(size, device=device) - 0.5) * math.sqrt(12)
    eps[0] = 0
    return eps


class Sampling(nn.Module):

    def __init__(self, latent_dim, sampling_size=1, sampling=True, distribution='gaussian', **kwargs):
        assert distribution in ('gaussian', 'uniform'), '{} for sampling unknown'.format(distribution)
        super().__init__(**kwargs)
        self.distribution = distribution
        self.sampling_size = sampling_size
        self.is_sampled = sampling

    def forward(self, z_mean, z_log_var, epsilon=None):
        K = z_mean.shape[-1]
        if epsilon is None:
            epsilon = draw_epsilon(self.sampling_size, z_log_var.shape, z_mean.device, self.distribution)
        mu2 = z_mean.reshape(-1, K)
        n = mu2.shape[0]
        labels = torch.zeros(n, dtype=torch.int64, device=z_mean.device)
        means = torch.zeros((1, K), device=z_mean.device)
        T = torch.ones(1, device=z_mean.device)
        _, z, _, _, _, _ = ops.latent(mu2, z_log_var.reshape(-1, K), epsilon.reshape(epsilon.shape[0], n, K), labels,
                                      means, T, sampled=bool(self.is_sampled))
        return z.reshape(epsilon.shape), epsilon[1:]

    def __repr__(self):
        if not self.is_sampled:
            return 'Deactivated, returns mean'
        return 'Sampling({}, L={})'.format(self.distribution, self.sampling_size)


class HipLinear(nn.Linear):

    def forward(self, x, act=ops.IDENT):
        return ops.linear(x, self.weight, self.bias, act)


class DenseStack(nn.Sequential):

    def forward(self, x):
        mods = list(self)
        i = 0
        while i < len(mods):
            m = mods[i]
            nxt = mods[i + 1] if i + 1 < len(mods) else None
            if isinstance(m, HipLinear) and type(nxt) in ACT_OF_MODULE:
                x = m(x, ACT_OF_MODULE[type(nxt)])
                i += 2
            else:
                x = m(x)
                i += 1
        return x


class HipDropout(nn.Module):

    _STRIDE = 0x9E3779B97F4A7C15 & (2 ** 62 - 1)

    def __init__(self, p=0.5):
        super().__init__()
        if not 0. <= p < 1.:
            raise ValueError('dropout probability has to be in [0, 1), got {}'.format(p))
        self.p = float(p)
        self._seed = None

    def _next_seed(self, device):
        if self._seed is None or self._seed.device != device:
            first = int(torch.randint(0, 2 ** 61, (1,)))
            if torch.distributed.is_available() and torch.distributed.is_initialized():
                first += torch.distributed.get_rank() * 1_000_003
            self._seed = torch.tensor([first], dtype=torch.int64, device=device)
        now = self._seed.clone()
        self._seed += self._STRIDE % (2 ** 31)
        return now

    def forward(self, x):
        if not self.training or self.p == 0.:
            if not x.is_cuda:
                raise ops.L.JvaeHipError('jvae_hip ops need tensors resident on the GPU (no CPU fallback)')
            return x
        return ops.dropout(x, self.p, self._next_seed(x.device))

    def extra_repr(self):
        return f'p={self.p}'


class Encoder(nn.Module):

    def __init__(self, input_shape, num_labels, representation='rgb', y_is_coded=False, latent_dim=32,
                 intermediate_dims=[64], name='encoder', dropout=False, activation='relu', sampling_size=10,
                 sampling=True, sigma_output_dim=0, forced_variance=False, prior={}, **kwargs):
        super().__init__(**kwargs)
        self.name = name
        self.y_is_coded = y_is_coded
        self.input_shape = input_shape
        self.num_labels = num_labels
        self.forced_variance = forced_variance
        self._sampling_size = sampling_size
        width = int(np.prod(input_shape)) + num_labels * bool(y_is_coded)
        trunk = []
        for d in intermediate_dims:
            trunk += [HipLinear(width, d), activation_layers[activation]()]
            if dropout:
                trunk.append(HipDropout(p=dropout))
            width = d
        self.dense_projs = DenseStack(*trunk)
        self.dense_mean = HipLinear(width, latent_dim)
        self.dense_log_var = HipLinear(width, latent_dim)
        self.sigma_output_dim = sigma_output_dim
        if sigma_output_dim:
            self.sigma = HipLinear(width, int(np.prod(sigma_output_dim)))

        noise = 'uniform' if prior.get('distribution', 'gaussian') == 'uniform' else 'gaussian'
        self.sampling = Sampling(latent_dim, sampling_size, sampling, distribution=noise)
        prior['dim'] = latent_dim
        self.prior = build_prior(**prior)
        logging.debug('Built %s', self.prior)
        self.mixed_prior = None

    @property
    def sampling_size(self):
        return self._sampling_size

    @sampling_size.setter
    def sampling_size(self, v):
        self._sampling_size = v
        self.sampling.sampling_size = v

    def capacity(self):
        m = self.prior.mean
        C = self.num_labels
        d2 = torch.cdist(m, m).pow(2)
        return math.log(C) - torch.exp(-d2 / 4).sum(0).log().sum() / C

    def dict_min_distance(self):
        m = self.prior.mean
        C = self.num_labels
        guard = 2 * m.norm(dim=1).max() * torch.eye(C, device=m.device)
        return (torch.cdist(m, m) + guard).min()

    def heads(self, x, y=None):
        u = x if y is None else torch.cat((x, y), dim=-1)
        u = self.dense_projs(u)
        return u, self.dense_mean(u), (None if self.forced_variance else self.dense_log_var(u))

    def encode(self, x, y_onehot, labels, kl_var_weighting=1., epsilon=None):
        u, mu, lv_raw = self.heads(x, y_onehot)
        K = mu.shape[-1]
        batch = mu.shape[:-1]
        mu2 = mu.reshape(-1, K)
        n = mu2.shape[0]
        pr = self.prior
        if epsilon is None:
            epsilon = draw_epsilon(self._sampling_size, mu.shape, mu.device, self.sampling.distribution)
        lab, means, T = pr._kernel_operands(labels if pr.conditional else None, n, mu.device)
        forced = math.log(self.forced_variance) if self.forced_variance else None
        raw2 = mu2 if lv_raw is None else lv_raw.reshape(-1, K)
        if self.mixed_prior is None:
            lv, z, kl, dist, vkl, dzd = ops.latent(mu2, raw2, epsilon.reshape(epsilon.shape[0], n, K), lab, means, T,
                                                   prior=pr.distribution, var_dim=pr.var_dim, tau=pr._tau,
                                                   alpha=pr._alpha_k, w=kl_var_weighting,
                                                   sampled=bool(self.sampling.is_sampled), forced_lv=forced)
        else:
            other, split = self.mixed_prior
            if not pr.conditional:
                raise NotImplementedError('a mixed prior needs the class-conditional prior in place')
            _, means_b, T_b = other._kernel_operands(labels if other.conditional else None, n, mu.device)
            describe = ops.latent_prior
            lv, z, kl, dist, vkl, dzd = ops.latent_mixed(
                mu2, raw2, epsilon.reshape(epsilon.shape[0], n, K), lab,
                describe(means, T, prior=pr.distribution, var_dim=pr.var_dim, tau=pr._tau, alpha=pr._alpha_k),
                describe(means_b, T_b, prior=other.distribution, var_dim=other.var_dim, tau=other._tau, alpha=other._alpha_k),
                split, w=kl_var_weighting, sampled=bool(self.sampling.is_sampled), forced_lv=forced)
        sigma = self.sigma(u) if self.sigma_output_dim else None
        terms = {'kl': kl.reshape(batch), 'distance': dist.reshape(batch), 'var_kl': vkl.reshape(batch),
                 'dzdist': dzd.reshape(batch)}
        return mu, lv.reshape(mu.shape), z.reshape(epsilon.shape), epsilon[1:], sigma, terms

    def forward(self, x, y=None, epsilon=None):
        labels = None
        if self.prior.conditional:
            labels = torch.zeros(x.shape[:-1], dtype=torch.int64, device=x.device)
        mu, log_var, z, e, sigma, _ = self.encode(x, y, labels, epsilon=epsilon)
        return mu, log_var, z, e, sigma


class Classifier(DenseStack):

    def __init__(self, latent_dim, num_labels, intermediate_dims=[], name='classifier', activation='relu', **kwargs):
        layers = []
        width = latent_dim
        act = activation_layers[activation]()
        for d in intermediate_dims:
            layers += [HipLinear(width, d), act]
            width = d
        layers.append(HipLinear(width, num_labels))
        super().__init__(*layers, **kwargs)
        self.name = name
```

Baseline: 142,700.

## Add grouped GEMM launch and fuse mean/log-var head linears into one pair op

Adds a grouped GEMM entry point that packs several independent GEMMs into one kernel launch, with each block finding its sub-problem from a prefix table, plus a grouped split-K fold. The encoder's mean and log-variance heads, which share an input, now go through a new paired linear autograd op whose forward and backward products are issued together as one grouped launch. The intent is to cut kernel-launch count and let small GEMMs fill the GPU at the same time. In exchange the grouped kernels carry a runtime variant switch, higher register/LDS pressure from the merged bodies, and an extra add to combine the two input gradients.

```diff
diff --git a/include/jvae_hip.h b/include/jvae_hip.h
--- a/include/jvae_hip.h
+++ b/include/jvae_hip.h
@@ -17,6 +17,22 @@
 
 int jvae_splitk_fold_f32(const float* part, const float* bias, float* y, int S, long MN, int N, int relu, int accumulate,
                          void* stream);
+
+typedef struct JvaeGemmDesc {
+    int M, N, K, batch;
+    const float* A; long sAm, sAk, sAb;
+    const float* B; long sBk, sBn, sBb;
+    float* C; long sCm, sCn, sCb;
+    const float* bias; int bias_mode, flags, splitk;
+    int want_splits; long sCsplit; int* splits;
+} JvaeGemmDesc;
+int jvae_gemm_group_f32(const JvaeGemmDesc* descs, int n, void* stream);
+
+typedef struct JvaeFoldDesc {
+    const float* part; const float* bias; float* y;
+    int S; long MN; int N, relu, accumulate;
+} JvaeFoldDesc;
+int jvae_splitk_fold_group_f32(const JvaeFoldDesc* descs, int n, void* stream);
 
 size_t jvae_conv2d_workspace_bytes(int N, int Cin, int H, int W, int Cout, int KH, int KW, int S, int P, int OP,
                                    int transposed);
diff --git a/joint-vae_amd/csrc/gemm.hip b/joint-vae_amd/csrc/gemm.hip
--- a/joint-vae_amd/csrc/gemm.hip
+++ b/joint-vae_amd/csrc/gemm.hip
@@ -1,5 +1,6 @@
 #include <stdlib.h>
 #include "common.h"
+#include "jvae_hip.h"
 #include "conv_x3.h"
 #include "jvae_internal.h"
 #include "conv_dispatch.h"
@@ -38,20 +39,28 @@
     return v;
 }
 
+template <int BM, int BN>
+struct TileLds {
+    static constexpr int LDA = BM + 4, LDB = BN + 4;
+    static constexpr int BYTES = BK * (LDA + LDB) * (int)sizeof(float);
+};
+
 template <int BM, int BN, bool AK, bool BNC>
-__global__ __launch_bounds__(256) void gemm_kernel(GemmP p) {
-    constexpr int LDA = BM + 4, LDB = BN + 4;
+__device__ __forceinline__ void gemm_tile_body(const GemmP& p, float* __restrict__ lds, unsigned bx, unsigned by, unsigned bz,
+                                               unsigned gx, unsigned gy, unsigned gz) {
+    constexpr int LDA = TileLds<BM, BN>::LDA, LDB = TileLds<BM, BN>::LDB;
     constexpr int WM = BM / 2, WN = BN / 2;
     constexpr int TM = WM / 32, TN = WN / 32;
     constexpr int GA = BM * BK / 4 / 256;
     constexpr int GB = BN * BK / 4 / 256;
-    __shared__ float As[BK * LDA];
-    __shared__ float Bs[BK * LDB];
+    float* As = lds;
+    float* Bs = lds + BK * LDA;
+    (void)gx; (void)gy; (void)gz;
 
     const int tid = threadIdx.x, lane = tid & 63, wave = tid >> 6;
     const int wm0 = (wave >> 1) * WM, wn0 = (wave & 1) * WN;
-    const int m0 = blockIdx.y * BM, n0 = blockIdx.x * BN;
-    const int batch = blockIdx.z / p.splitk, split = blockIdx.z % p.splitk;
+    const int m0 = by * BM, n0 = bx * BN;
+    const int batch = bz / p.splitk, split = bz % p.splitk;
     const int kbeg = split * p.kchunk;
     const int kend = min(p.K, kbeg + p.kchunk);
     const float* A = p.A + (long)batch * p.sAb;
@@ -177,16 +186,10 @@
         }
 }
 
-template <int BM, int BN>
-int launch_tile(const GemmP& p, int batch, hipStream_t st) {
-    dim3 grid(cdiv(p.N, BN), cdiv(p.M, BM), batch * p.splitk), block(256);
-    const bool ak = (p.sAk == 1), bnc = (p.sBn == 1);
-    if (ak && bnc)       hipLaunchKernelGGL((gemm_kernel<BM, BN, true, true>), grid, block, 0, st, p);
-    else if (ak && !bnc) hipLaunchKernelGGL((gemm_kernel<BM, BN, true, false>), grid, block, 0, st, p);
-    else if (!ak && bnc) hipLaunchKernelGGL((gemm_kernel<BM, BN, false, true>), grid, block, 0, st, p);
-    else                 hipLaunchKernelGGL((gemm_kernel<BM, BN, false, false>), grid, block, 0, st, p);
-    JVAE_LAUNCH_CHECK();
-    return 0;
+template <int BM, int BN, bool AK, bool BNC>
+__global__ __launch_bounds__(256) void gemm_kernel(GemmP p) {
+    __shared__ float lds[TileLds<BM, BN>::BYTES / sizeof(float)];
+    gemm_tile_body<BM, BN, AK, BNC>(p, lds, blockIdx.x, blockIdx.y, blockIdx.z, gridDim.x, gridDim.y, gridDim.z);
 }
 
 inline bool aligned16(const void* p) { return (reinterpret_cast<uintptr_t>(p) & 15) == 0; }
@@ -214,13 +217,13 @@
     static constexpr int BYTES = PITCH * ROWS;
 };
 
-template <bool AK, bool BNC, int DEPTH = 1>
-__global__ __launch_bounds__(256, 4) void gemm_x3_kernel(GemmP p) {
+template <bool AK, bool BNC, int DEPTH>
+__device__ __forceinline__ void gemm_x3_body(const GemmP& p, unsigned char* __restrict__ gx_lds, unsigned bx, unsigned by, unsigned bz,
+                                             unsigned gx, unsigned gy, unsigned gz) {
     using IA = GxImg<AK>;
     using IB = GxImg<!BNC>;
     constexpr int BM = 64, BN = 64, G4 = BM * BKX / 4 / 256;
     constexpr int KQX = BKX / 4;
-    extern __shared__ __attribute__((aligned(16))) unsigned char gx_lds[];
     unsigned char* As = gx_lds;
     unsigned char* Bs = gx_lds + 3 * IA::BYTES;
 
@@ -228,10 +231,9 @@
     const int half = lane >> 5, l31 = lane & 31;
     const int cg = (lane >> 4) & 1, q4 = (lane & 15) >> 2, pp = lane & 3;
     const int wm0 = (wave >> 1) * 32, wn0 = (wave & 1) * 32;
-    unsigned bx = blockIdx.x, by = blockIdx.y, bz = blockIdx.z;
     if (p.xcd) {
-        const unsigned lin = (unsigned)xcd_tile(bx + gridDim.x * (by + gridDim.y * bz), gridDim.x * gridDim.y * gridDim.z);
-        bx = lin % gridDim.x; by = (lin / gridDim.x) % gridDim.y; bz = lin / (gridDim.x * gridDim.y);
+        const unsigned lin = (unsigned)xcd_tile(bx + gx * (by + gy * bz), gx * gy * gz);
+        bx = lin % gx; by = (lin / gx) % gy; bz = lin / (gx * gy);
     }
     const int m0 = by * BM, n0 = bx * BN;
     const int batch = bz / p.splitk, split = bz % p.splitk;
@@ -400,43 +402,286 @@
     }
 }
 
-template <bool AK, bool BNC, int DEPTH>
-int launch_x3_variant(const GemmP& p, int batch, hipStream_t st) {
-    constexpr int LDS = 3 * (GxImg<AK>::BYTES + GxImg<!BNC>::BYTES);
-    static bool attr_set = false;
-    if (!attr_set) {
-        hipError_t e = hipFuncSetAttribute(reinterpret_cast<const void*>(&gemm_x3_kernel<AK, BNC, DEPTH>),
-                                           hipFuncAttributeMaxDynamicSharedMemorySize, LDS);
+template <bool AK, bool BNC, int DEPTH = 1>
+__global__ __launch_bounds__(256, 4) void gemm_x3_kernel(GemmP p) {
+    extern __shared__ __attribute__((aligned(16))) unsigned char gx_lds[];
+    gemm_x3_body<AK, BNC, DEPTH>(p, gx_lds, blockIdx.x, blockIdx.y, blockIdx.z, gridDim.x, gridDim.y, gridDim.z);
+}
+
+inline bool gemm_x3_on(int K) {
+    return K >= 64 && jvae_conv5_x3_enabled();
+}
+
+constexpr int VAR_X3 = 8;
+struct GemmPlan {
+    GemmP p;
+    int variant;
+    unsigned gx, gy, gz;
+    int lds;
+};
+
+template <bool AK, bool BNC>
+constexpr int x3_lds() { return 3 * (GxImg<AK>::BYTES + GxImg<!BNC>::BYTES); }
+
+inline int variant_lds(int v) {
+    if (v < 4) return TileLds<64, 64>::BYTES;
+    if (v < VAR_X3) return TileLds<128, 128>::BYTES;
+    switch ((v - VAR_X3) >> 1) {
+        case 0: return x3_lds<false, false>();
+        case 1: return x3_lds<false, true>();
+        case 2: return x3_lds<true, false>();
+        default: return x3_lds<true, true>();
+    }
+}
+
+struct GemmArgs {
+    int M, N, K, batch;
+    const float* A; long sAm, sAk, sAb;
+    const float* B; long sBk, sBn, sBb;
+    float* C; long sCm, sCn, sCb;
+    const float* bias; int bias_mode, bias_div, flags, splitk;
+    int part;
+    long sCsplit;
+};
+
+int gemm_plan(const GemmArgs& a, GemmPlan* pl) {
+    if (a.M <= 0 || a.N <= 0 || a.batch <= 0) return 1;
+    if (!a.A || !a.B || !a.C) return JVAE_EINVAL;
+    if (a.part ? a.K <= 0 : a.K < 0) return JVAE_EINVAL;
+    if (!a.part && a.bias_mode && !a.bias) return JVAE_EINVAL;
+    GemmP& p = pl->p;
+    p.A = a.A; p.sAm = a.sAm; p.sAk = a.sAk; p.sAb = a.sAb;
+    p.B = a.B; p.sBk = a.sBk; p.sBn = a.sBn; p.sBb = a.sBb;
+    p.C = a.C; p.sCm = a.sCm; p.sCn = a.sCn; p.sCb = a.sCb;
+    p.bias = a.part ? nullptr : a.bias;
+    p.bias_mode = a.part ? 0 : a.bias_mode;
+    p.bias_div = (!a.part && a.bias_div > 0) ? a.bias_div : 1;
+    p.M = a.M; p.N = a.N; p.K = a.K;
+    int splitk = a.splitk < 1 ? 1 : a.splitk;
+    const int ktiles = cdiv(a.K, BK);
+    if (splitk > ktiles) splitk = ktiles > 0 ? ktiles : 1;
+    p.kchunk = cdiv(ktiles, splitk) * BK;
+    splitk = a.K > 0 ? cdiv(a.K, p.kchunk) : 1;
+    p.splitk = splitk;
+    if (a.part) {
+        p.flags = 8;
+        p.sCsplit = a.sCsplit;
+    } else {
+        p.flags = a.flags & ~8;
+        p.sCsplit = 0;
+        if (splitk > 1) {
+            if (a.flags & 2) return JVAE_EINVAL;
+            p.flags |= 4;
+        }
+    }
+    const bool ak = (a.sAk == 1), bnc = (a.sBn == 1);
+    p.vecA = aligned16(a.A) && (a.sAb % 4 == 0) && (ak ? (a.sAm % 4 == 0) : (a.sAm == 1 && a.sAk % 4 == 0));
+    p.vecB = aligned16(a.B) && (a.sBb % 4 == 0) && (bnc ? (a.sBk % 4 == 0) : (a.sBk == 1 && a.sBn % 4 == 0));
+    p.xcd = 0;
+    int bm = 64;
+    if (gemm_x3_on(a.K)) {
+        p.xcd = 1;
+        const bool deep = p.vecA && p.vecB && p.K % 4 == 0 && (ak || p.M % 4 == 0) && (!bnc || p.N % 4 == 0);
+        pl->variant = VAR_X3 + 4 * ak + 2 * bnc + (deep ? 1 : 0);
+    } else {
+        const long tiles128 = (long)cdiv(a.M, 128) * cdiv(a.N, 128) * a.batch * splitk;
+        if (!a.part && a.M > 64 && a.N > 64 && tiles128 >= 512) bm = 128;
+        pl->variant = (bm == 128 ? 4 : 0) + 2 * ak + (bnc ? 1 : 0);
+    }
+    pl->gx = cdiv(a.N, bm); pl->gy = cdiv(a.M, bm); pl->gz = (unsigned)a.batch * splitk;
+    pl->lds = variant_lds(pl->variant);
+    return 0;
+}
+
+template <typename F>
+int set_lds_once(F kernel, int lds, bool* done) {
+    if (!*done) {
+        hipError_t e = hipFuncSetAttribute(reinterpret_cast<const void*>(kernel), hipFuncAttributeMaxDynamicSharedMemorySize, lds);
         if (e != hipSuccess) return (int)e;
-        attr_set = true;
-    }
-    dim3 grid(cdiv(p.N, 64), cdiv(p.M, 64), batch * p.splitk), block(256);
-    hipLaunchKernelGGL((gemm_x3_kernel<AK, BNC, DEPTH>), grid, block, LDS, st, p);
+        *done = true;
+    }
+    return 0;
+}
+
+template <int BM, bool AK, bool BNC>
+int launch_tile_variant(const GemmPlan& pl, hipStream_t st) {
+    hipLaunchKernelGGL((gemm_kernel<BM, BM, AK, BNC>), dim3(pl.gx, pl.gy, pl.gz), dim3(256), 0, st, pl.p);
     JVAE_LAUNCH_CHECK();
     return 0;
 }
 
-template <bool AK, bool BNC>
-int launch_x3_ab(const GemmP& p, int batch, hipStream_t st) {
-    const bool deep = p.vecA && p.vecB && p.K % 4 == 0
-                      && (AK || p.M % 4 == 0) && (!BNC || p.N % 4 == 0);
-    if (deep) return launch_x3_variant<AK, BNC, 3>(p, batch, st);
-    return launch_x3_variant<AK, BNC, 1>(p, batch, st);
-}
-
-int launch_x3(const GemmP& p0, int batch, hipStream_t st) {
-    GemmP p = p0;
-    p.xcd = 1;
-    const bool ak = (p.sAk == 1), bnc = (p.sBn == 1);
-    if (ak && bnc) return launch_x3_ab<true, true>(p, batch, st);
-    if (ak) return launch_x3_ab<true, false>(p, batch, st);
-    if (bnc) return launch_x3_ab<false, true>(p, batch, st);
-    return launch_x3_ab<false, false>(p, batch, st);
-}
-
-inline bool gemm_x3_on(int K) {
-    return K >= 64 && jvae_conv5_x3_enabled();
-}
+template <bool AK, bool BNC, int DEPTH>
+int launch_x3_variant(const GemmPlan& pl, hipStream_t st) {
+    static bool attr_set = false;
+    if (int rc = set_lds_once(&gemm_x3_kernel<AK, BNC, DEPTH>, x3_lds<AK, BNC>(), &attr_set)) return rc;
+    hipLaunchKernelGGL((gemm_x3_kernel<AK, BNC, DEPTH>), dim3(pl.gx, pl.gy, pl.gz), dim3(256), pl.lds, st, pl.p);
+    JVAE_LAUNCH_CHECK();
+    return 0;
+}
+
+int launch_plan(const GemmPlan& pl, hipStream_t st) {
+    switch (pl.variant) {
+        case 0: return launch_tile_variant<64, false, false>(pl, st);
+        case 1: return launch_tile_variant<64, false, true>(pl, st);
+        case 2: return launch_tile_variant<64, true, false>(pl, st);
+        case 3: return launch_tile_variant<64, true, true>(pl, st);
+        case 4: return launch_tile_variant<128, false, false>(pl, st);
+        case 5: return launch_tile_variant<128, false, true>(pl, st);
+        case 6: return launch_tile_variant<128, true, false>(pl, st);
+        case 7: return launch_tile_variant<128, true, true>(pl, st);
+        case 8: return launch_x3_variant<false, false, 1>(pl, st);
+        case 9: return launch_x3_variant<false, false, 3>(pl, st);
+        case 10: return launch_x3_variant<false, true, 1>(pl, st);
+        case 11: return launch_x3_variant<false, true, 3>(pl, st);
+        case 12: return launch_x3_variant<true, false, 1>(pl, st);
+        case 13: return launch_x3_variant<true, false, 3>(pl, st);
+        case 14: return launch_x3_variant<true, true, 1>(pl, st);
+        case 15: return launch_x3_variant<true, true, 3>(pl, st);
+    }
+    return JVAE_EINVAL;
+}
+
+constexpr int GROUP_MAX = 8;
+struct GemmRec {
+    GemmP p;
+    int variant;
+    unsigned gx, gy, gz;
+    unsigned first;
+};
+struct GemmGroup {
+    GemmRec rec[GROUP_MAX];
+};
+
+struct GroupTile { unsigned r, bx, by, bz; bool live; };
+__device__ __forceinline__ GroupTile group_tile(const GemmGroup& g) {
+    unsigned r = 0;
+#pragma unroll
+    for (unsigned i = 1; i < GROUP_MAX; ++i)
+        if (blockIdx.x >= g.rec[i].first) r = i;
+    const GemmRec& rc = g.rec[r];
+    const unsigned local = blockIdx.x - rc.first;
+    GroupTile t;
+    t.r = r;
+    t.live = local < rc.gx * rc.gy * rc.gz;
+    t.bx = local % rc.gx; t.by = (local / rc.gx) % rc.gy; t.bz = local / (rc.gx * rc.gy);
+    return t;
+}
+
+template <bool BIG>
+__global__ __launch_bounds__(256) void gemm_group_tile_kernel(GemmGroup g) {
+    extern __shared__ __attribute__((aligned(16))) unsigned char grp_lds[];
+    float* lds = reinterpret_cast<float*>(grp_lds);
+    const GroupTile t = group_tile(g);
+    if (!t.live) return;
+    const GemmRec& rc = g.rec[t.r];
+    switch (rc.variant) {
+        case 0: gemm_tile_body<64, 64, false, false>(rc.p, lds, t.bx, t.by, t.bz, rc.gx, rc.gy, rc.gz); return;
+        case 1: gemm_tile_body<64, 64, false, true>(rc.p, lds, t.bx, t.by, t.bz, rc.gx, rc.gy, rc.gz); return;
+        case 2: gemm_tile_body<64, 64, true, false>(rc.p, lds, t.bx, t.by, t.bz, rc.gx, rc.gy, rc.gz); return;
+        case 3: gemm_tile_body<64, 64, true, true>(rc.p, lds, t.bx, t.by, t.bz, rc.gx, rc.gy, rc.gz); return;
+    }
+    if constexpr (BIG) {
+        switch (rc.variant) {
+            case 4: gemm_tile_body<128, 128, false, false>(rc.p, lds, t.bx, t.by, t.bz, rc.gx, rc.gy, rc.gz); return;
+            case 5: gemm_tile_body<128, 128, false, true>(rc.p, lds, t.bx, t.by, t.bz, rc.gx, rc.gy, rc.gz); return;
+            case 6: gemm_tile_body<128, 128, true, false>(rc.p, lds, t.bx, t.by, t.bz, rc.gx, rc.gy, rc.gz); return;
+            case 7: gemm_tile_body<128, 128, true, true>(rc.p, lds, t.bx, t.by, t.bz, rc.gx, rc.gy, rc.gz); return;
+        }
+    }
+}
+
+template <bool BIG>
+int launch_group_tile(const GemmGroup& g, unsigned total, int lds, hipStream_t st) {
+    static bool attr_set = false;
+    if (int rc = set_lds_once(&gemm_group_tile_kernel<BIG>, TileLds<BIG ? 128 : 64, BIG ? 128 : 64>::BYTES, &attr_set)) return rc;
+    hipLaunchKernelGGL(gemm_group_tile_kernel<BIG>, dim3(total), dim3(256), lds, st, g);
+    JVAE_LAUNCH_CHECK();
+    return 0;
+}
+
+constexpr unsigned X3_FWD = 1u << (13 - VAR_X3), X3_BWD = (1u << (15 - VAR_X3)) | (1u << (11 - VAR_X3)), X3_ALL = 0xffu;
+
+template <unsigned MASK, int V, bool AK, bool BNC, int DEPTH>
+__device__ __forceinline__ void group_x3_case(const GemmRec& rc, unsigned char* lds, const GroupTile& t) {
+    if constexpr ((MASK >> (V - VAR_X3)) & 1u) {
+        if (rc.variant == V) gemm_x3_body<AK, BNC, DEPTH>(rc.p, lds, t.bx, t.by, t.bz, rc.gx, rc.gy, rc.gz);
+    }
+}
+
+template <unsigned MASK>
+__global__ __launch_bounds__(256, 4) void gemm_group_x3_kernel(GemmGroup g) {
+    extern __shared__ __attribute__((aligned(16))) unsigned char grp_lds[];
+    const GroupTile t = group_tile(g);
+    if (!t.live) return;
+    const GemmRec& rc = g.rec[t.r];
+    group_x3_case<MASK, 8, false, false, 1>(rc, grp_lds, t);
+    group_x3_case<MASK, 9, false, false, 3>(rc, grp_lds, t);
+    group_x3_case<MASK, 10, false, true, 1>(rc, grp_lds, t);
+    group_x3_case<MASK, 11, false, true, 3>(rc, grp_lds, t);
+    group_x3_case<MASK, 12, true, false, 1>(rc, grp_lds, t);
+    group_x3_case<MASK, 13, true, false, 3>(rc, grp_lds, t);
+    group_x3_case<MASK, 14, true, true, 1>(rc, grp_lds, t);
+    group_x3_case<MASK, 15, true, true, 3>(rc, grp_lds, t);
+}
+
+template <unsigned MASK>
+int launch_group_x3(const GemmGroup& g, unsigned total, int lds, hipStream_t st) {
+    static bool attr_set = false;
+    if (int rc = set_lds_once(&gemm_group_x3_kernel<MASK>, x3_lds<false, false>(), &attr_set)) return rc;
+    hipLaunchKernelGGL(gemm_group_x3_kernel<MASK>, dim3(total), dim3(256), lds, st, g);
+    JVAE_LAUNCH_CHECK();
+    return 0;
+}
+
+int launch_group_kind(const GemmPlan* plans, int n, bool x3, hipStream_t st) {
+    GemmGroup g;
+    int cnt = 0, lds = 0, last = -1;
+    unsigned long total = 0;
+    for (int i = 0; i < n; ++i) {
+        if ((plans[i].variant >= VAR_X3) != x3) continue;
+        GemmRec& rc = g.rec[cnt++];
+        rc.p = plans[i].p; rc.variant = plans[i].variant;
+        rc.gx = plans[i].gx; rc.gy = plans[i].gy; rc.gz = plans[i].gz;
+        rc.first = (unsigned)total;
+        total += ((unsigned long)rc.gx * rc.gy * rc.gz + 7) & ~7ul;
+        if (total > 0x7fffffffUL) return JVAE_ENOTSUP;
+        if (plans[i].lds > lds) lds = plans[i].lds;
+        last = i;
+    }
+    if (cnt == 0) return 0;
+    if (cnt == 1) return launch_plan(plans[last], st);
+    for (int i = cnt; i < GROUP_MAX; ++i) { g.rec[i] = g.rec[0]; g.rec[i].first = 0xffffffffu; }
+    if (x3) {
+        unsigned mask = 0;
+        for (int i = 0; i < cnt; ++i) mask |= 1u << (g.rec[i].variant - VAR_X3);
+        if ((mask & ~X3_FWD) == 0) return launch_group_x3<X3_FWD>(g, (unsigned)total, lds, st);
+        if ((mask & ~X3_BWD) == 0) return launch_group_x3<X3_BWD>(g, (unsigned)total, lds, st);
+        return launch_group_x3<X3_ALL>(g, (unsigned)total, lds, st);
+    }
+    for (int i = 0; i < cnt; ++i)
+        if (g.rec[i].variant >= 4) return launch_group_tile<true>(g, (unsigned)total, lds, st);
+    return launch_group_tile<false>(g, (unsigned)total, lds, st);
+}
+
+int launch_group(const GemmPlan* plans, int n, hipStream_t st) {
+    if (int rc = launch_group_kind(plans, n, true, st)) return rc;
+    return launch_group_kind(plans, n, false, st);
+}
+
+void plan_out_range(const GemmPlan& pl, uintptr_t* lo, uintptr_t* hi) {
+    const GemmP& p = pl.p;
+    const long batch = pl.gz / p.splitk;
+    long neg = 0, pos = 0;
+    auto span = [&](long stride, long count) {
+        const long d = stride * (count - 1);
+        if (d < 0) neg += d; else pos += d;
+    };
+    span(p.sCm, p.M); span(p.sCn, p.N); span(p.sCb, batch);
+    if (p.flags & 8) span(p.sCsplit, p.splitk);
+    *lo = reinterpret_cast<uintptr_t>(p.C + neg);
+    *hi = reinterpret_cast<uintptr_t>(p.C + pos) + sizeof(float) - 1;
+}
+
 
 }
 
@@ -454,34 +699,12 @@
                         const float* B, long sBk, long sBn, long sBb,
                         float* C, long sCm, long sCn, long sCb,
                         const float* bias, int bias_mode, int bias_div, int flags, int splitk, hipStream_t st) {
-    if (M <= 0 || N <= 0 || batch <= 0) return 0;
-    if (K < 0 || !A || !B || !C) return JVAE_EINVAL;
-    if (bias_mode && !bias) return JVAE_EINVAL;
-    GemmP p;
-    p.A = A; p.sAm = sAm; p.sAk = sAk; p.sAb = sAb;
-    p.B = B; p.sBk = sBk; p.sBn = sBn; p.sBb = sBb;
-    p.C = C; p.sCm = sCm; p.sCn = sCn; p.sCb = sCb;
-    p.bias = bias; p.bias_mode = bias_mode; p.bias_div = bias_div > 0 ? bias_div : 1;
-    p.M = M; p.N = N; p.K = K;
-    if (splitk < 1) splitk = 1;
-    int ktiles = cdiv(K, BK);
-    if (splitk > ktiles) splitk = ktiles > 0 ? ktiles : 1;
-    p.kchunk = cdiv(ktiles, splitk) * BK;
-    splitk = K > 0 ? cdiv(K, p.kchunk) : 1;
-    p.splitk = splitk;
-    p.flags = flags & ~8;
-    p.sCsplit = 0;
-    if (splitk > 1) {
-        if (flags & 2) return JVAE_EINVAL;
-        p.flags |= 4;
-    }
-    const bool ak = (sAk == 1), bnc = (sBn == 1);
-    p.vecA = aligned16(A) && (sAb % 4 == 0) && (ak ? (sAm % 4 == 0) : (sAm == 1 && sAk % 4 == 0));
-    p.vecB = aligned16(B) && (sBb % 4 == 0) && (bnc ? (sBk % 4 == 0) : (sBk == 1 && sBn % 4 == 0));
-    if (gemm_x3_on(K)) return launch_x3(p, batch, st);
-    const long tiles128 = (long)cdiv(M, 128) * cdiv(N, 128) * batch * splitk;
-    if (M > 64 && N > 64 && tiles128 >= 512) return launch_tile<128, 128>(p, batch, st);
-    return launch_tile<64, 64>(p, batch, st);
+    const GemmArgs a = {M, N, K, batch, A, sAm, sAk, sAb, B, sBk, sBn, sBb, C, sCm, sCn, sCb,
+                        bias, bias_mode, bias_div, flags, splitk, 0, 0};
+    GemmPlan pl;
+    const int rc = gemm_plan(a, &pl);
+    if (rc) return rc < 0 ? rc : 0;
+    return launch_plan(pl, st);
 }
 
 int jvae_gemm_launch_part(int M, int N, int K, int batch,
@@ -490,40 +713,84 @@
                           float* part, long sCm, long sCn, long sCb, long sCsplit, int want_splits, int* splits,
                           hipStream_t st) {
     if (splits) *splits = 0;
-    if (M <= 0 || N <= 0 || batch <= 0) return 0;
-    if (K <= 0 || !A || !B || !part || !splits) return JVAE_EINVAL;
-    GemmP p;
-    p.A = A; p.sAm = sAm; p.sAk = sAk; p.sAb = sAb;
-    p.B = B; p.sBk = sBk; p.sBn = sBn; p.sBb = sBb;
-    p.C = part; p.sCm = sCm; p.sCn = sCn; p.sCb = sCb;
-    p.bias = nullptr; p.bias_mode = 0; p.bias_div = 1;
-    p.M = M; p.N = N; p.K = K;
-    int splitk = want_splits < 1 ? 1 : want_splits;
-    const int ktiles = cdiv(K, BK);
-    if (splitk > ktiles) splitk = ktiles;
-    p.kchunk = cdiv(ktiles, splitk) * BK;
-    splitk = cdiv(K, p.kchunk);
-    p.splitk = splitk;
-    p.flags = 8;
-    p.sCsplit = sCsplit;
-    const bool ak = (sAk == 1), bnc = (sBn == 1);
-    p.vecA = aligned16(A) && (sAb % 4 == 0) && (ak ? (sAm % 4 == 0) : (sAm == 1 && sAk % 4 == 0));
-    p.vecB = aligned16(B) && (sBb % 4 == 0) && (bnc ? (sBk % 4 == 0) : (sBk == 1 && sBn % 4 == 0));
-    *splits = splitk;
-    if (gemm_x3_on(K)) return launch_x3(p, batch, st);
-    return launch_tile<64, 64>(p, batch, st);
-}
-
-__global__ __launch_bounds__(256) void splitk_fold_kernel(const float* __restrict__ part, const float* __restrict__ bias,
-                                                          float* __restrict__ y, int S, long MN, int N, int relu,
-                                                          int accumulate, int bias_div) {
-    for (long i = (long)blockIdx.x * blockDim.x + threadIdx.x; i < MN; i += (long)gridDim.x * blockDim.x) {
+    const GemmArgs a = {M, N, K, batch, A, sAm, sAk, sAb, B, sBk, sBn, sBb, part, sCm, sCn, sCb,
+                        nullptr, 0, 1, 0, want_splits, 1, sCsplit};
+    GemmPlan pl;
+    const int rc = gemm_plan(a, &pl);
+    if (rc) return rc < 0 ? rc : 0;
+    if (!splits) return JVAE_EINVAL;
+    *splits = pl.p.splitk;
+    return launch_plan(pl, st);
+}
+
+extern "C" int jvae_gemm_group_f32(const JvaeGemmDesc* descs, int n, void* stream) {
+    if (n == 0) return 0;
+    if (n < 0 || !descs) return JVAE_EINVAL;
+    if (n > GROUP_MAX) return JVAE_ENOTSUP;
+    GemmPlan plans[GROUP_MAX];
+    uintptr_t lo[GROUP_MAX], hi[GROUP_MAX];
+    int cnt = 0;
+    for (int i = 0; i < n; ++i) {
+        const JvaeGemmDesc& d = descs[i];
+        if (d.splits) *d.splits = 0;
+        const bool part = d.want_splits > 0;
+        const GemmArgs a = {d.M, d.N, d.K, d.batch, d.A, d.sAm, d.sAk, d.sAb, d.B, d.sBk, d.sBn, d.sBb, d.C, d.sCm, d.sCn, d.sCb,
+                            d.bias, d.bias_mode, 1, d.flags, part ? d.want_splits : d.splitk, part ? 1 : 0, d.sCsplit};
+        const int rc = gemm_plan(a, &plans[cnt]);
+        if (rc < 0) return rc;
+        if (rc) continue;
+        if (part && !d.splits) return JVAE_EINVAL;
+        plan_out_range(plans[cnt], &lo[cnt], &hi[cnt]);
+        for (int j = 0; j < cnt; ++j)
+            if (lo[cnt] <= hi[j] && lo[j] <= hi[cnt]) return JVAE_EINVAL;
+        ++cnt;
+    }
+    for (int i = 0, k = 0; i < n; ++i) {
+        const JvaeGemmDesc& d = descs[i];
+        if (d.M <= 0 || d.N <= 0 || d.batch <= 0) continue;
+        if (d.splits) *d.splits = plans[k].p.splitk;
+        ++k;
+    }
+    return launch_group(plans, cnt, (hipStream_t)stream);
+}
+
+__device__ __forceinline__ void splitk_fold_body(const float* __restrict__ part, const float* __restrict__ bias, float* __restrict__ y,
+                                                 int S, long MN, int N, int relu, int accumulate, int bias_div, unsigned block,
+                                                 unsigned blocks) {
+    for (long i = (long)block * blockDim.x + threadIdx.x; i < MN; i += (long)blocks * blockDim.x) {
         float v = bias ? bias[(i / bias_div) % N] : 0.f;
         for (int s = 0; s < S; ++s) v += part[(long)s * MN + i];
         if (accumulate) v += y[i];
         y[i] = relu ? fmaxf(v, 0.f) : v;
     }
 }
+
+__global__ __launch_bounds__(256) void splitk_fold_kernel(const float* __restrict__ part, const float* __restrict__ bias,
+                                                          float* __restrict__ y, int S, long MN, int N, int relu,
+                                                          int accumulate, int bias_div) {
+    splitk_fold_body(part, bias, y, S, MN, N, relu, accumulate, bias_div, blockIdx.x, gridDim.x);
+}
+
+struct FoldRec {
+    const float* part; const float* bias; float* y;
+    long MN;
+    int S, N, relu, accumulate, bias_div;
+    unsigned first, blocks;
+};
+struct FoldGroup {
+    FoldRec rec[8];
+};
+
+__global__ __launch_bounds__(256) void splitk_fold_group_kernel(FoldGroup g) {
+    unsigned r = 0;
+#pragma unroll
+    for (unsigned i = 1; i < 8; ++i)
+        if (blockIdx.x >= g.rec[i].first) r = i;
+    const FoldRec& rc = g.rec[r];
+    splitk_fold_body(rc.part, rc.bias, rc.y, rc.S, rc.MN, rc.N, rc.relu, rc.accumulate, rc.bias_div, blockIdx.x - rc.first, rc.blocks);
+}
+
+inline int fold_blocks(long MN) { return (int)((MN + 255) / 256 > 4096 ? 4096 : (MN + 255) / 256); }
 
 __global__ __launch_bounds__(256) void splitk_fold_qn_kernel(const float* __restrict__ part, const float* __restrict__ bias,
                                                              float* __restrict__ y, int S, int N, int Cs, int Ps) {
@@ -550,7 +817,7 @@
 int jvae_splitk_fold(const float* part, const float* bias, float* y, int S, long MN, int N, int relu, int accumulate,
                      hipStream_t st, int bias_div) {
     if (MN == 0) return 0;
-    const int blocks = (int)((MN + 255) / 256 > 4096 ? 4096 : (MN + 255) / 256);
+    const int blocks = fold_blocks(MN);
     hipLaunchKernelGGL(splitk_fold_kernel, dim3(blocks), dim3(256), 0, st, part, bias, y, S, MN, N, relu, accumulate,
                        bias_div > 0 ? bias_div : 1);
     JVAE_LAUNCH_CHECK();
@@ -561,6 +828,39 @@
                                     int accumulate, void* stream) {
     if (!part || !y || S < 1 || MN < 0 || N < 1) return JVAE_EINVAL;
     return jvae_splitk_fold(part, bias, y, S, MN, N, relu, accumulate, (hipStream_t)stream);
+}
+
+extern "C" int jvae_splitk_fold_group_f32(const JvaeFoldDesc* descs, int n, void* stream) {
+    if (n == 0) return 0;
+    if (n < 0 || !descs) return JVAE_EINVAL;
+    if (n > 8) return JVAE_ENOTSUP;
+    FoldGroup g;
+    int cnt = 0, last = -1;
+    unsigned total = 0;
+    for (int i = 0; i < n; ++i) {
+        const JvaeFoldDesc& d = descs[i];
+        if (!d.part || !d.y || d.S < 1 || d.MN < 0 || d.N < 1) return JVAE_EINVAL;
+        for (int j = 0; j < i; ++j) {
+            const JvaeFoldDesc& e = descs[j];
+            if (d.MN > 0 && e.MN > 0 && d.y < e.y + e.MN && e.y < d.y + d.MN) return JVAE_EINVAL;
+        }
+        if (d.MN == 0) continue;
+        FoldRec& rc = g.rec[cnt++];
+        rc.part = d.part; rc.bias = d.bias; rc.y = d.y; rc.MN = d.MN;
+        rc.S = d.S; rc.N = d.N; rc.relu = d.relu; rc.accumulate = d.accumulate; rc.bias_div = 1;
+        rc.first = total; rc.blocks = (unsigned)fold_blocks(d.MN);
+        total += rc.blocks;
+        last = i;
+    }
+    if (cnt == 0) return 0;
+    if (cnt == 1) {
+        const JvaeFoldDesc& d = descs[last];
+        return jvae_splitk_fold(d.part, d.bias, d.y, d.S, d.MN, d.N, d.relu, d.accumulate, (hipStream_t)stream);
+    }
+    for (int i = cnt; i < 8; ++i) { g.rec[i] = g.rec[0]; g.rec[i].first = 0xffffffffu; }
+    hipLaunchKernelGGL(splitk_fold_group_kernel, dim3(total), dim3(256), 0, (hipStream_t)stream, g);
+    JVAE_LAUNCH_CHECK();
+    return 0;
 }
 
 extern "C" int jvae_gemm_f32(int M, int N, int K, int batch,
diff --git a/joint-vae_amd/jvae_hip/lib.py b/joint-vae_amd/jvae_hip/lib.py
--- a/joint-vae_amd/jvae_hip/lib.py
+++ b/joint-vae_amd/jvae_hip/lib.py
@@ -10,10 +10,28 @@
 _lib = None
 
 P = c_void_p
+
+
+class GemmDesc(ctypes.Structure):
+    _fields_ = ([('M', c_int), ('N', c_int), ('K', c_int), ('batch', c_int)]
+                + [('A', P), ('sAm', c_long), ('sAk', c_long), ('sAb', c_long)]
+                + [('B', P), ('sBk', c_long), ('sBn', c_long), ('sBb', c_long)]
+                + [('C', P), ('sCm', c_long), ('sCn', c_long), ('sCb', c_long)]
+                + [('bias', P), ('bias_mode', c_int), ('flags', c_int), ('splitk', c_int)]
+                + [('want_splits', c_int), ('sCsplit', c_long), ('splits', POINTER(c_int))])
+
+
+class FoldDesc(ctypes.Structure):
+    _fields_ = [('part', P), ('bias', P), ('y', P), ('S', c_int), ('MN', c_long), ('N', c_int), ('relu', c_int),
+                ('accumulate', c_int)]
+
+
 _SIGS = {
     'jvae_version': (c_char_p, []),
     'jvae_gemm_f32': (c_int, [c_int] * 4 + [P, c_long, c_long, c_long] * 3 + [P, c_int, c_int, c_int, P]),
     'jvae_splitk_fold_f32': (c_int, [P, P, P, c_int, c_long, c_int, c_int, c_int, P]),
+    'jvae_gemm_group_f32': (c_int, [POINTER(GemmDesc), c_int, P]),
+    'jvae_splitk_fold_group_f32': (c_int, [POINTER(FoldDesc), c_int, P]),
     'jvae_conv2d_workspace_bytes': (c_size_t, [c_int] * 11),
     'jvae_conv2d_set_split_bf16': (c_int, [c_int]),
     'jvae_conv2d_set_split_shape16': (c_int, [c_int]),
diff --git a/joint-vae_amd/jvae_hip/ops.py b/joint-vae_amd/jvae_hip/ops.py
--- a/joint-vae_amd/jvae_hip/ops.py
+++ b/joint-vae_amd/jvae_hip/ops.py
@@ -48,6 +48,45 @@
     rc = lib.jvae_gemm_f32(M, N, K, batch, L.ptr(A), *sA, L.ptr(B), *sB, L.ptr(C), *sC,
                            L.ptr(bias), bias_mode, flags, splitk, L.stream_ptr())
     L.check(rc, 'jvae_gemm_f32')
+
+
+def gemm_desc(M, N, K, A, sA, B, sB, C, sC, bias=None, bias_mode=0, flags=0, splitk=1, batch=1):
+    return (M, N, K, batch, A, sA, B, sB, C, sC, bias, bias_mode, flags, splitk)
+
+
+def gemm_group(descs):
+    lib = L.load()
+    arr = (L.GemmDesc * max(len(descs), 1))()
+    for d, (M, N, K, batch, A, sA, B, sB, C, sC, bias, bias_mode, flags, splitk) in zip(arr, descs):
+        d.M, d.N, d.K, d.batch = M, N, K, batch
+        d.A, (d.sAm, d.sAk, d.sAb) = L.ptr(A), sA
+        d.B, (d.sBk, d.sBn, d.sBb) = L.ptr(B), sB
+        d.C, (d.sCm, d.sCn, d.sCb) = L.ptr(C), sC
+        d.bias, d.bias_mode, d.flags, d.splitk = L.ptr(bias), bias_mode, flags, splitk
+    L.check(lib.jvae_gemm_group_f32(arr, len(descs), L.stream_ptr()), 'jvae_gemm_group_f32')
+
+
+def splitk_fold_group(jobs):
+    lib = L.load()
+    arr = (L.FoldDesc * max(len(jobs), 1))()
+    for d, (part, bias, y, S, MN, N, relu, accumulate) in zip(arr, jobs):
+        d.part, d.bias, d.y = L.ptr(part), L.ptr(bias), L.ptr(y)
+        d.S, d.MN, d.N, d.relu, d.accumulate = S, MN, N, relu, accumulate
+    L.check(lib.jvae_splitk_fold_group_f32(arr, len(jobs), L.stream_ptr()), 'jvae_splitk_fold_group_f32')
+
+
+def _run_products(descs, folds):
+    if len(descs) == 1:
+        M, N, K, batch, A, sA, B, sB, C, sC, bias, bias_mode, flags, splitk = descs[0]
+        gemm(M, N, K, A, sA, B, sB, C, sC, bias=bias, bias_mode=bias_mode, flags=flags, splitk=splitk, batch=batch)
+    elif descs:
+        gemm_group(descs)
+    if len(folds) == 1:
+        part, bias, y, S, MN, N, relu, accumulate = folds[0]
+        L.check(L.load().jvae_splitk_fold_f32(L.ptr(part), L.ptr(bias), L.ptr(y), S, MN, N, relu, accumulate, L.stream_ptr()),
+                'jvae_splitk_fold_f32')
+    elif folds:
+        splitk_fold_group(folds)
 
 
 def channel_sum(t, N, C, P, out=None, accumulate=False):
@@ -110,36 +149,117 @@
             g = torch.empty_like(gy)
             L.check(lib.jvae_act_bwd_f32(L.ptr(gy), L.ptr(y), L.ptr(g), gy.numel(), ctx.act, L.stream_ptr()), 'act_bwd')
             gy = g
-        gx = gw = gb = None
-        if ctx.needs_input_grad[0]:
-            gx = torch.empty((R, I), device=gy.device, dtype=torch.float32)
-            gemm(R, I, O, gy, (O, 1, 0), w, (I, 1, 0), gx, (I, 1, 0))
+        descs, folds = [], []
+        gx, gw = _linear_bwd_products(gy, x2, w, ctx.w_ref, ctx.needs_input_grad[0], ctx.needs_input_grad[1], descs, folds)
+        _run_products(descs, folds)
+        if gx is not None:
             gx = gx.reshape(ctx.xshape)
-        if ctx.needs_input_grad[1]:
-            slot = _grad_slot(ctx.w_ref)
-            gw = slot if slot is not None else torch.zeros((O, I), device=gy.device, dtype=torch.float32)
-            S = _linear_split(O, I, R)
-            if S > 1:
-                part = torch.empty((S, O, I), device=gy.device, dtype=torch.float32)
-                Rs = R // S
-                gemm(O, I, Rs, gy, (1, O, Rs * O), x2, (I, 1, Rs * I), part, (I, 1, O * I), batch=S)
-                L.check(lib.jvae_splitk_fold_f32(L.ptr(part), None, L.ptr(gw), S, O * I, I, 0, 1, L.stream_ptr()),
-                        'jvae_splitk_fold_f32')
-            else:
-                gemm(O, I, R, gy, (1, O, 0), x2, (I, 1, 0), gw, (I, 1, 0), flags=1)
-            if slot is not None:
-                gw = None
-        if ctx.has_bias and ctx.needs_input_grad[2]:
-            slot = _grad_slot(ctx.b_ref)
-            if slot is not None:
-                channel_sum(gy, R, O, 1, out=slot, accumulate=True)
-            else:
-                gb = channel_sum(gy, R, O, 1)
+        gb = _linear_bias_grad(gy, ctx.b_ref) if ctx.has_bias and ctx.needs_input_grad[2] else None
         return gx, gw, gb, None
+
+
+def _linear_fwd_products(x2, w, b, act, descs, folds):
+    R, I = x2.shape
+    O = w.shape[0]
+    y = torch.empty((R, O), device=x2.device, dtype=torch.float32)
+    S = _linear_split(R, O, I)
+    if S > 1:
+        part = torch.empty((S, R, O), device=x2.device, dtype=torch.float32)
+        Ks = I // S
+        descs.append(gemm_desc(R, O, Ks, x2, (I, 1, Ks), w, (1, I, Ks), part, (O, 1, R * O), batch=S))
+        folds.append((part, b, y, S, R * O, O, int(act == RELU), 0))
+    else:
+        descs.append(gemm_desc(R, O, I, x2, (I, 1, 0), w, (1, I, 0), y, (O, 1, 0), bias=b, bias_mode=1 if b is not None else 0,
+                               flags=2 if act == RELU else 0))
+    return y
+
+
+def _linear_bwd_products(gy, x2, w, w_ref, need_x, need_w, descs, folds):
+    R, I = x2.shape
+    O = w.shape[0]
+    gx = gw = None
+    if need_x:
+        gx = torch.empty((R, I), device=gy.device, dtype=torch.float32)
+        descs.append(gemm_desc(R, I, O, gy, (O, 1, 0), w, (I, 1, 0), gx, (I, 1, 0)))
+    if need_w:
+        slot = _grad_slot(w_ref)
+        gw = slot if slot is not None else torch.zeros((O, I), device=gy.device, dtype=torch.float32)
+        S = _linear_split(O, I, R)
+        if S > 1:
+            part = torch.empty((S, O, I), device=gy.device, dtype=torch.float32)
+            Rs = R // S
+            descs.append(gemm_desc(O, I, Rs, gy, (1, O, Rs * O), x2, (I, 1, Rs * I), part, (I, 1, O * I), batch=S))
+            folds.append((part, None, gw, S, O * I, I, 0, 1))
+        else:
+            descs.append(gemm_desc(O, I, R, gy, (1, O, 0), x2, (I, 1, 0), gw, (I, 1, 0), flags=1))
+        if slot is not None:
+            gw = None
+    return gx, gw
+
+
+def _linear_bias_grad(gy, b_ref):
+    R, O = gy.shape
+    slot = _grad_slot(b_ref)
+    if slot is not None:
+        channel_sum(gy, R, O, 1, out=slot, accumulate=True)
+        return None
+    return channel_sum(gy, R, O, 1)
 
 
 def linear(x, w, b=None, act=IDENT):
     return _Linear.apply(x, w, b, act)
+
+
+class _LinearPair(torch.autograd.Function):
+
+    @staticmethod
+    def forward(ctx, x, w0, b0, w1, b1):
+        x2 = _c(_f32(x, 'linear_pair').reshape(-1, x.shape[-1]))
+        ws = (_c(w0), _c(w1))
+        descs, folds = [], []
+        ys = [_linear_fwd_products(x2, w, b, IDENT, descs, folds) for w, b in zip(ws, (b0, b1))]
+        _run_products(descs, folds)
+        ctx.save_for_backward(x2, *ws)
+        ctx.xshape = x.shape
+        ctx.refs = ((w0, b0), (w1, b1))
+        ctx.set_materialize_grads(False)
+        return tuple(y.reshape(*x.shape[:-1], y.shape[1]) for y in ys)
+
+    @staticmethod
+    def backward(ctx, g0, g1):
+        x2, *ws = ctx.saved_tensors
+        R = x2.shape[0]
+        descs, folds = [], []
+        out = []
+        gxs = []
+        gys = []
+        for h, g in enumerate((g0, g1)):
+            if g is None:
+                out += [None, None]
+                gys.append(None)
+                continue
+            gy = _c(g.reshape(R, ws[h].shape[0]))
+            gx, gw = _linear_bwd_products(gy, x2, ws[h], ctx.refs[h][0], ctx.needs_input_grad[0], ctx.needs_input_grad[1 + 2 * h],
+                                          descs, folds)
+            if gx is not None:
+                gxs.append(gx)
+            out += [gw, None]
+            gys.append(gy)
+        _run_products(descs, folds)
+        for h, gy in enumerate(gys):
+            b_ref = ctx.refs[h][1]
+            if gy is not None and b_ref is not None and ctx.needs_input_grad[2 + 2 * h]:
+                out[1 + 2 * h] = _linear_bias_grad(gy, b_ref)
+        gx = None
+        if gxs:
+            gx = (gxs[0] if len(gxs) == 1 else torch.add(gxs[0], gxs[1])).reshape(ctx.xshape)
+        return (gx, *out)
+
+
+def linear_pair(x, w0, b0, w1, b1):
+    if w0 is w1:
+        return linear(x, w0, b0), linear(x, w1, b1)
+    return _LinearPair.apply(x, w0, b0, w1, b1)
 
 
 _GEOM_CACHE = {}
diff --git a/joint-vae_amd/module/vae_layers/layers.py b/joint-vae_amd/module/vae_layers/layers.py
--- a/joint-vae_amd/module/vae_layers/layers.py
+++ b/joint-vae_amd/module/vae_layers/layers.py
@@ -284,7 +284,10 @@
     def heads(self, x, y=None):
         u = x if y is None else torch.cat((x, y), dim=-1)
         u = self.dense_projs(u)
-        return u, self.dense_mean(u), (None if self.forced_variance else self.dense_log_var(u))
+        if self.forced_variance:
+            return u, self.dense_mean(u), None
+        mu, lv = ops.linear_pair(u, self.dense_mean.weight, self.dense_mean.bias, self.dense_log_var.weight, self.dense_log_var.bias)
+        return u, mu, lv
 
     def encode(self, x, y_onehot, labels, kl_var_weighting=1., epsilon=None):
         u, mu, lv_raw = self.heads(x, y_onehot)
```

Measured after the change: 144,100, median of 6. 1.01x the previous value.
